# vr308/Generalised-Gaussian-Processes

Measured on AMD Instinct MI355X. Metric: ELBO evals/sec, higher is better.
Workload: dtype f64

## Files before the change

### generalised-gaussian-processes_amd/_lib.py

```python
from __future__ import annotations

import ctypes as C
import os

HERE = os.path.dirname(os.path.abspath(__file__))
LIB_PATH = os.path.join(HERE, "csrc", "libsgp_hip.so")

SGP_ABI_VERSION = 3
SGP_MAX_DIM = 32
SGP_MAX_INDUCING = 4096
KERNEL_IDS = {"rbf": 0, "matern32": 1, "matern52": 2, "composite": 3}
LIKELIHOOD_IDS = {"gaussian": 0, "bernoulli": 1, "bernoulli_logit": 2, "poisson": 3}
SGPMC_LIK_OUT_LEN = 3
COMP_LEN = 33
OPT_CONTRACTION, OPT_ASM_OVERLAP, OPT_KFU_BUDGET_BYTES, OPT_COND_LIMIT, OPT_CU_BUDGET, OPT_TIMING, OPT_SHARED_DEVICE = range(7)
OUT_F, OUT_LOGMARG, OUT_TRACE, OUT_LOGDETB, OUT_QUAD, OUT_TRW, OUT_S2BAR, OUT_KAPPABAR, OUT_LEN = range(9)


class SgpLibraryError(RuntimeError):
    pass


class SgpStatusError(RuntimeError):
    def __init__(self, fn, status, text):
        super().__init__("%s returned %d: %s" % (fn, status, text))
        self.status = status


_vp, _i64, _i32, _dbl, _sz = C.c_void_p, C.c_int64, C.c_int, C.c_double, C.c_size_t
_dp = C.POINTER(C.c_double)
_ip = C.POINTER(C.c_int)

PROTOTYPES = {
    "sgp_abi_version": (_i32, []),
    "sgp_status_string": (C.c_char_p, [_i32]),
    "sgp_ctx_create": (_vp, [_i32]),
    "sgp_ctx_destroy": (None, [_vp]),
    "sgp_ctx_device": (_i32, [_vp]),
    "sgp_ctx_set_option": (_i32, [_vp, _i32, _dbl]),
    "sgp_ctx_get_option": (_dbl, [_vp, _i32]),
    "sgp_ctx_bind_thread": (None, [_vp]),
    "sgp_ctx_set_pass1_gate": (None, [_vp, _vp]),
    "sgp_ctx_contraction_last": (_i32, [_vp]),
    "sgp_ctx_contraction_would_use_i8": (_i32, [_vp, _i64, _i32]),
    "sgp_ctx_timing_last_ms": (_i32, [_vp, _i32, C.POINTER(C.c_float)]),
    "sgp_ctx_timing_last_rows": (_i64, [_vp, _i32]),
    "sgp_ctx_suffstats_workspace_bytes": (_sz, [_vp, _i64, _i32, _i32, _i32]),
    "sgp_ctx_suffstats_fwd": (_i32, [_vp, _vp, _i64, _vp, _vp, _i64, _dp, _dbl, _i64, _i32, _i32, _i32,
                                     _vp, _vp, _vp, _vp, _vp, _vp, _sz, _vp]),
    "sgp_ctx_suffstats_bwd": (_i32, [_vp, _vp, _i64, _vp, _vp, _i64, _dp, _dbl, _vp, _vp, _dbl, _vp, _i64, _i32, _i32, _i32,
                                     _vp, _vp, _vp, _vp, _sz, _vp]),
    "sgp_ctx_kuu_factor": (_i32, [_vp, _vp, _i32, _vp, _vp, _vp, _sz, _vp]),
    "sgp_ctx_kuu_factor_ex": (_i32, [_vp, _vp, _i32, _vp, _vp, _vp, _vp, _sz, _vp]),
    "sgp_ctx_bound_from_stats": (_i32, [_vp, _vp, _vp, _vp, _vp, _vp, _dbl, _i64, _i32, _i32, _vp,
                                        _vp, _vp, _vp, _vp, _vp, _vp, _vp, _sz, _vp]),
    "sgp_ctx_suffstats_whitened_workspace_bytes": (_sz, [_vp, _i64, _i32, _i32]),
    "sgp_ctx_suffstats_fwd_whitened": (_i32, [_vp, _vp, _i64, _vp, _vp, _i64, _dp, _dbl, _i64, _i32, _i32, _i32, _vp,
                                              _vp, _vp, _vp, _vp, _vp, _sz, _vp]),
    "sgp_ctx_suffstats_whitened_rows_workspace_bytes": (_sz, [_vp, _i64, _i32, _i32, _i32]),
    "sgp_ctx_suffstats_fwd_whitened_rows": (_i32, [_vp, _vp, _i64, _vp, _vp, _i64, _dp, _dbl, _i64, _i32, _i32, _i32, _vp,
                                                   _vp, _vp, _vp, _vp, _vp, _vp, _sz, _vp]),
    "sgp_ctx_suffstats_extended_workspace_bytes": (_sz, [_vp, _i64, _i32, _i32]),
    "sgp_ctx_suffstats_fwd_extended": (_i32, [_vp, _vp, _i64, _vp, _vp, _i64, _dp, _dbl, _i64, _i32, _i32, _i32, _vp, _i32,
                                              _vp, _vp, _vp, _vp, _vp, _vp, _vp, _sz, _vp]),
    "sgp_ctx_suffstats_fwd_extended_f16": (_i32, [_vp, _vp, _i64, _vp, _vp, _i64, _dp, _dbl, _i64, _i32, _i32, _i32, _vp, _i32,
                                                  _vp, _vp, _vp, _vp, _vp, _vp, _vp, _vp, _sz, _vp]),
    "sgp_ctx_suffstats_bwd_factored_workspace_bytes": (_sz, [_vp, _i64, _i32, _i32, _i32]),
    "sgp_ctx_suffstats_bwd_factored": (_i32, [_vp, _vp, _i64, _vp, _vp, _i64, _dp, _dbl, _vp, _vp, _dbl, _vp, _dbl, _i64, _i32, _i32, _i32,
                                              _vp, _vp, _vp, _vp, _vp, _sz, _vp]),
    "sgp_ctx_bound_from_whitened_stats": (_i32, [_vp, _vp, _vp, _vp, _vp, _dbl, _i64, _i32, _i32, _vp,
                                                 _vp, _vp, _vp, _vp, _vp, _vp, _vp, _vp, _sz, _vp]),
    "sgp_ctx_mixture_predict": (_i32, [_vp, _vp, _i64, _vp, _i64, _vp, _i64, _i64, _vp, _i64, _i32, _dp, _dp, _dp, _dbl, _i32, _i32, _i32, _i32,
                                       _dbl, _vp, _vp, _vp, _vp, _vp, _vp, _sz, _vp]),
    "sgp_ctx_mixture_predict_zs": (_i32, [_vp, _vp, _i64, _vp, _i64, _vp, _i64, _i64, _vp, _i64, _i64, _i32, _dp, _dp, _dp, _dbl, _i32, _i32, _i32, _i32, _dbl, _vp, _vp, _vp, _vp, _vp, _vp, _sz, _vp]),
    "sgp_timing_enable": (None, [_i32]),
    "sgp_timing_last_ms": (_i32, [_i32, C.POINTER(C.c_float)]),
    "sgp_timing_last_rows": (_i64, [_i32]),
    "sgp_set_asm_overlap": (None, [_i32]),
    "sgp_set_cond_limit": (None, [_dbl]),
    "sgp_suffstats_workspace_bytes": (_sz, [_i64, _i32, _i32]),
    "sgp_suffstats_workspace_bytes_ex": (_sz, [_i64, _i32, _i32, _i32]),
    "sgp_suffstats_bwd_workspace_bytes_ex": (_sz, [_i64, _i32, _i32, _i32]),
    "sgp_kfu_len": (_sz, [_i64, _i32]),
    "sgp_set_kfu_budget_bytes": (None, [_sz]),
    "sgp_set_contraction": (_i32, [_i32]),
    "sgp_contraction_last": (_i32, []),
    "sgp_set_pass1_gate": (None, [_vp]),
    "sgp_suffstats_fwd": (_i32, [_vp, _i64, _vp, _vp, _i64, _dp, _dbl, _i64, _i32, _i32, _i32,
                                 _vp, _vp, _vp, _vp, _vp, _vp, _sz, _vp]),
    "sgp_stats_packed_len": (_sz, [_i32]),
    "sgp_stats_pack_lower": (_i32, [_vp, _i32, _vp, _vp]),
    "sgp_stats_unpack_lower": (_i32, [_vp, _i32, _vp, _vp]),
    "sgp_kuu": (_i32, [_vp, _i64, _dp, _dbl, _dbl, _i32, _i32, _i32, _vp, _vp]),
    "sgp_chol_workspace_bytes": (_sz, [_i32]),
    "sgp_chol_lower": (_i32, [_vp, _i64, _i32, _vp, _vp, _sz, _vp]),
    "sgp_trsm_workspace_bytes": (_sz, [_i32, _i32]),
    "sgp_trsm_lower": (_i32, [_vp, _i64, _vp, _i64, _i32, _i32, _i32, _vp, _sz, _vp]),
    "sgp_logdiag_sum": (_i32, [_vp, _i64, _i32, _vp, _vp]),
# ... 145 lines not shown
```

### generalised-gaussian-processes_amd/core.py

```python
from __future__ import annotations

import math

import torch

try:
    import torch.distributed as dist
except Exception:
    dist = None

from ._lib import COMP_LEN, OUT_F, OUT_LOGMARG, OUT_S2BAR, OUT_TRACE


class NotPositiveDefiniteError(RuntimeError):

    def __init__(self, info):
        super().__init__("matrix not positive definite: leading minor of order %d (1..M: Kuu, M+1..2M: B)" % info)
        self.info = info


class SgpTimeoutError(RuntimeError):

    def __init__(self):
        super().__init__("device time-out inside the dataflow Cholesky (SGP_INFO_TIMEOUT): outputs are invalid")
# ... 290 lines not shown
        if tier == TIER_WHITENED:
            self.guard.note_bound(ub, tol)
            return None
        need = required_tier(est, tol, reach, ext_ok)
        self.guard.note_exact(est, ub, tol)
        if need > tier:
            self.guard.open = True
            return need
        if info != 0:
            return tier + 1 if (tier + 1 < TIER_WHITENED and ext_ok) else TIER_WHITENED
        if strict and need < tier:
            return need
        return None

    def _forward(self, Z, ls, sf2, s2, with_adjoints, want_factors=False, extra=0, tier=TIER_STREAMING, report=False, want_lo=True):
        e = self.engine
        M = int(Z.shape[0])
        result = e.result_buffer(extra)
        if tier == TIER_EXTENDED:
            self.n_extended += 1
            Kuu = e.kuu(Z, ls, sf2, self.jitter, self.kernel)
            linv, _ = e.kuu_factor(Kuu, info=result[2], trace_out=self._trace_buf() if report else None)
            kfu = self._kfu_for(M) if with_adjoints else None
            diag = None
            if report:
                if self._phi_diag is None or self._phi_diag.numel() < M:
                    self._phi_diag = e.empty(M)
                diag = self._phi_diag
            dd = with_adjoints and self.extended_dd_phibar and hasattr(e, "phibar_dd")
            lo = dd and want_lo and kfu is not None and self._bwd_lo_ok(M)
            kfu_f16 = self._kfu_f16_for(M) if lo else None
            packed = e.suffstats_extended(self.X, self.y, Z, ls, sf2, linv, self.kernel, kfu=kfu, level=self.extended_level,
                                          **({"phi_diag": diag} if diag is not None else {}), **({"kfu_f16": kfu_f16} if kfu_f16 is not None else {}))
            self._allreduce_stats(packed, M)
            res = e.bound(Kuu, packed, s2, self.N, with_adjoints=with_adjoints, want_factors=want_factors, kuu_linv=linv,
                          result=result, whitened=True, **({"want_cw": True} if dd else {}))
            if dd:
                res["Phibar"], res["Phibar_lo"] = e.phibar_dd(res["Cw"], linv, s2, want_lo=lo)
                res["Cw"] = None
            if report:
                self._allreduce(diag[:M])
                e.streaming_error_report(diag, 1, self._trace_buf(), sf2, s2, self.N, M, result)
                res["reported"] = True
            res.update(packed=packed, kfu=kfu, kfu_f16=kfu_f16, t_keep=None, linv=linv)
            return res
        if tier == TIER_WHITENED:
            Kuu = e.kuu(Z, ls, sf2, self.jitter, self.kernel)
            rep = report and self.kernel != "composite"
            linv, _ = e.kuu_factor(Kuu, info=result[2], trace_out=self._trace_buf() if rep else None)
            factored = with_adjoints and self.factored_adjoint and hasattr(e, "suffstats_bwd_factored")
            t_keep = None
            if whitened_rows_layout(e, self.kernel, int(self.X.shape[0]), M, self.whitened_rows_min_work):
                t_keep = self._kfu_for(M) if factored else None
                packed = e.suffstats_whitened_rows(self.X, self.y, Z, ls, sf2, linv, self.kernel, t_out=t_keep)
            else:
                packed = e.suffstats_whitened(self.X, self.y, Z, ls, sf2, linv, self.kernel)
            self._allreduce_stats(packed, M)
            kw = {"want_cw": True} if factored else {}
            res = e.bound(Kuu, packed, s2, self.N, with_adjoints=with_adjoints, want_factors=want_factors, kuu_linv=linv,
                          result=result, whitened=True, **kw)
            if rep:
                e.streaming_error_report(None, 1, self._trace_buf(), sf2, s2, self.N, M, result)
                res["reported"] = True
            res.update(packed=packed, kfu=None, t_keep=t_keep, linv=linv)
            return res
        kfu = self._kfu_for(M) if with_adjoints else None
        gate = None
        guard = report
        trace = self._trace_buf() if guard and hasattr(e, "kuu_factor") else None
        overlap = (self.overlap_tail and hasattr(e, "kuu_factor") and e.device.type == "cuda"
                   and int(self.X.shape[0]) * M >= self.overlap_min_work)
        if overlap:
            main = torch.cuda.current_stream(e.device)
            side, (z_ready, ready), (Kuu, linv) = self._side_state(M)
            z_ready.record(main)
            side.wait_event(z_ready)
            e.kuu(Z, ls, sf2, self.jitter, self.kernel, out=Kuu, stream=side)
            e.kuu_factor(Kuu, info=result[2], trace_out=trace, out=linv, stream=side)
            ready.record(side)
            if (hasattr(e, "would_use_i8") and self.kernel != "composite" and int(self.X.shape[0]) >= 300 * M
                    and e.would_use_i8(int(self.X.shape[0]), M)):
                gate = ready
        try:
            packed = e.suffstats(self.X, self.y, Z, ls, sf2, self.kernel, kfu=kfu, **({"gate": gate} if gate is not None else {}))
            self._allreduce_stats(packed, M)
        finally:
            if overlap:
                main.wait_event(ready)
        if overlap:
            res = e.bound(Kuu, packed, s2, self.N, with_adjoints=with_adjoints, want_factors=want_factors, kuu_linv=linv,
                          result=result)
        elif guard and hasattr(e, "kuu_factor"):
            Kuu = e.kuu(Z, ls, sf2, self.jitter, self.kernel)
            linv, _ = e.kuu_factor(Kuu, info=result[2], trace_out=trace)
            res = e.bound(Kuu, packed, s2, self.N, with_adjoints=with_adjoints, want_factors=want_factors, kuu_linv=linv,
                          result=result)
        else:
            Kuu = e.kuu(Z, ls, sf2, self.jitter, self.kernel)
            res = e.bound(Kuu, packed, s2, self.N, with_adjoints=with_adjoints, want_factors=want_factors, result=result)
        if guard and trace is not None:
            e.streaming_error_report(packed, M + 1, trace, sf2, s2, self.N, M, result)
            res["reported"] = True
        res["packed"] = packed
        res["kfu"] = kfu
        return res

    def _pass2(self, res, Z, ls, sf2, s2, want_gz, g):
        e = self.engine
        if res.get("Cw") is not None:
            e.suffstats_bwd_factored(self.X, self.y, Z, ls, sf2, res["linv"], res["Cw"], s2, res["bbar"], -1.0 / (2.0 * float(s2)),
                                     self.kernel, want_gz=want_gz, out=g,
                                     **({"t_in": res["t_keep"]} if res.get("t_keep") is not None else {}))
        else:
            e.suffstats_bwd(self.X, self.y, Z, ls, sf2, res["Phibar"], res["bbar"], -1.0 / (2.0 * float(s2)),
                            self.kernel, want_gz=want_gz, out=g, kfu=res["kfu"])
            if res.get("Phibar_lo") is not None:
                n_lo = int(res.get("lo_slots", 0))
                e.suffstats_bwd_lo(self.X, self.y, Z, ls, sf2, res["Phibar_lo"], res["kfu"], g, self.kernel,
                                   **({"delta": g[g.numel() - n_lo:]} if n_lo else {}),
                                   **({"kfu_f16": res["kfu_f16"]} if res.get("kfu_f16") is not None else {}))
        if int(res.get("lo_slots", 0)) and res.get("Phibar_lo") is None:
            g[g.numel() - int(res["lo_slots"]):].zero_()
        self._allreduce(g)
        e.kuu_bwd(Z, ls, sf2, res["Kuubar"], g, self.kernel, want_gz=want_gz)

    def _evaluate(self, *args, **kw):
        try:
            return self._evaluate_once(*args, **kw)
        except SgpTimeoutError:
            e = self.engine
            if "shared_device" not in getattr(e, "OPTIONS", {}) or e.get_option("shared_device") != 0:
                raise
            e.set_option("shared_device", 1)
            self.n_timeout_retries += 1
            return self._evaluate_once(*args, **kw)

    def _evaluate_once(self, Z, ls, sf2, s2, with_grad=False, want_gz=False, want_factors=False, grad_reach=None, strict=False):
        e = self.engine
        M, d = int(Z.shape[0]), int(Z.shape[1])
        guard = self._guard_on(M)
        reach = self.extended_range
        if with_grad:
            reach = float(grad_reach) if grad_reach is not None else (self.extended_grad_range_lo if self._bwd_lo_ok(M) else self.extended_grad_range)
        ext_ok = self._extended_ok(M)
        if guard:
            tier = self.guard.start_tier(self.streaming_tol, reach, ext_ok)
            if strict and tier == TIER_WHITENED:
                tier = TIER_EXTENDED if ext_ok else TIER_STREAMING
            if tier != TIER_STREAMING:
                self.n_direct_whitened += 1
        else:
            tier = self._fixed_tier(M)
        nh = (e.hyper_len(self.kernel, d) if hasattr(e, "hyper_len") else d) if with_grad else 0
        lo_slots = (nh + 1) if (with_grad and guard and ext_ok and self._bwd_lo_ok(M)) else 0
        extra = nh + 1 + (M * d if want_gz else 0) + lo_slots if with_grad else 0
        if guard and with_grad and tier == TIER_EXTENDED and grad_reach is None and self._lo_skip > 0:
            self._lo_skip -= 1
            tier = TIER_WHITENED
        early = with_grad and self._rows_for_form * M >= self.early_check_min_work
        done = {}
        may_go_down = strict
        while True:
            res = self._forward(Z, ls, sf2, s2, with_adjoints=with_grad, want_factors=want_factors, extra=extra, tier=tier, report=guard,
                                want_lo=grad_reach is None)
            head = res["buf"].numel() - extra
            g = res["buf"][head:] if with_grad else None
            res["lo_slots"] = lo_slots
# ... 129 lines not shown
```

### generalised-gaussian-processes_amd/csrc/sgp_ctx.hip

```cpp
#include "sgp_common.hpp"
#include "sgp_ctx.hpp"
#include "sgp_stream.hpp"
#include <cstdlib>
#include <new>

namespace sgp {

static void ctx_init(Ctx& c, int device) {
  c.device = device;
  c.contraction = env_int("SGP_CONTRACTION", 1);
  if (c.contraction < 0 || c.contraction > 2) c.contraction = 1;
  c.asm_overlap = env_int("SGP_ASM_OVERLAP", 0);
  c.kfu_budget = KFU_BUDGET_DEFAULT;
  c.syrk_skip_upper = env_int("SGP_SYRK_SKIP_UPPER", 1);
  c.syrk_waves = env_int("SGP_SYRK_WAVES", 4);
  c.syrk_glds = env_int("SGP_SYRK_GLDS", 0);
  c.i8_prio = env_int("SGP_I8_PRIO", 0);
  c.shared_device = env_int("SGP_SHARED_DEVICE", 0) != 0 ? 1 : 0;
}

Ctx& default_ctx() {
  static Ctx* c = [] {
    Ctx* p = new Ctx();
    int dev = 0;
    if (hipGetDevice(&dev) != hipSuccess) dev = 0;
    ctx_init(*p, dev);
    return p;
  }();
  return *c;
}

static thread_local Ctx* t_cur = nullptr;
static thread_local Ctx* t_bound = nullptr;
Ctx& cur_ctx() { return t_cur ? *t_cur : (t_bound ? *t_bound : default_ctx()); }
void bind_thread_ctx(void* ctx) { t_bound = static_cast<Ctx*>(ctx); }
CtxScope::CtxScope(void* ctx) : prev(t_cur) { t_cur = ctx ? static_cast<Ctx*>(ctx) : &default_ctx(); }
CtxScope::~CtxScope() { t_cur = prev; }

}

using namespace sgp;

static bool ctx_on_current_device(const sgp_ctx* ctx) {
  if (!ctx) return true;
  int dev = -1;
  if (hipGetDevice(&dev) != hipSuccess) return true;
  return dev == reinterpret_cast<const Ctx*>(ctx)->device;
}

extern "C" sgp_ctx* sgp_ctx_create(int device) {
  if (device < 0) return nullptr;
  Ctx* c = new (std::nothrow) Ctx();
  if (!c) return nullptr;
  ctx_init(*c, device);
  return reinterpret_cast<sgp_ctx*>(c);
}

extern "C" void sgp_ctx_destroy(sgp_ctx* ctx) {
  if (!ctx) return;
  Ctx* c = reinterpret_cast<Ctx*>(ctx);
  if (c == &default_ctx()) return;
  if (c->ev_ready)
    for (int s = 0; s < CTX_TIMING_SLOTS; ++s)
      for (int k = 0; k < 2; ++k) (void)hipEventDestroy(c->ev[s][k]);
  if (c->side) {
    (void)hipStreamDestroy(c->side);
    (void)hipEventDestroy(c->ev_fork);
    (void)hipEventDestroy(c->ev_join);
  }
  delete c;
}

extern "C" int sgp_ctx_set_option(sgp_ctx* ctx, int option, double value) {
  Ctx& c = ctx ? *reinterpret_cast<Ctx*>(ctx) : default_ctx();
  switch (option) {
    case SGP_OPT_CONTRACTION:
      if (!(value >= 0.0 && value <= 2.0)) return SGP_ERR_ARG;
      c.contraction = (int)value;
      return SGP_OK;
    case SGP_OPT_ASM_OVERLAP:
      if (!(value >= 0.0 && value <= 2.0)) return SGP_ERR_ARG;
      c.asm_overlap = (int)value;
      return SGP_OK;
    case SGP_OPT_KFU_BUDGET_BYTES:
      if (!(value >= 0.0)) return SGP_ERR_ARG;
      c.kfu_budget = value > 0.0 ? (size_t)value : KFU_BUDGET_DEFAULT;
      return SGP_OK;
    case SGP_OPT_COND_LIMIT:
      c.cond_limit = value >= 0.0 ? value : 1e13;
      return SGP_OK;
    case SGP_OPT_CU_BUDGET:
      c.cu_budget = value > 0.0 ? (int)value : 0;
      return SGP_OK;
    case SGP_OPT_TIMING:
      c.timing = value != 0.0 ? 1 : 0;
      return SGP_OK;
    case SGP_OPT_SHARED_DEVICE:
      c.shared_device = value != 0.0 ? 1 : 0;
      return SGP_OK;
    default:
      return SGP_ERR_ARG;
  }
}

extern "C" double sgp_ctx_get_option(const sgp_ctx* ctx, int option) {
  const Ctx& c = ctx ? *reinterpret_cast<const Ctx*>(ctx) : default_ctx();
  switch (option) {
    case SGP_OPT_CONTRACTION: return (double)c.contraction;
    case SGP_OPT_ASM_OVERLAP: return (double)c.asm_overlap;
    case SGP_OPT_KFU_BUDGET_BYTES: return (double)c.kfu_budget;
    case SGP_OPT_COND_LIMIT: return c.cond_limit;
    case SGP_OPT_CU_BUDGET: return (double)c.cu_budget;
    case SGP_OPT_TIMING: return (double)c.timing;
    case SGP_OPT_SHARED_DEVICE: return (double)c.shared_device;
    default: return -1.0;
  }
}

extern "C" void sgp_ctx_bind_thread(sgp_ctx* ctx) { sgp::bind_thread_ctx(ctx); }

extern "C" int sgp_ctx_device(const sgp_ctx* ctx) { return (ctx ? *reinterpret_cast<const Ctx*>(ctx) : default_ctx()).device; }

extern "C" void sgp_ctx_set_pass1_gate(sgp_ctx* ctx, void* hip_event) {
  (ctx ? *reinterpret_cast<Ctx*>(ctx) : default_ctx()).pass1_gate = (hipEvent_t)hip_event;
}

extern "C" int sgp_ctx_contraction_last(const sgp_ctx* ctx) {
  return (ctx ? *reinterpret_cast<const Ctx*>(ctx) : default_ctx()).contraction_used;
}

extern "C" size_t sgp_ctx_suffstats_workspace_bytes(const sgp_ctx* ctx, int64_t N, int M, int d, int caller_owns_kfu) {
  CtxScope scope(const_cast<sgp_ctx*>(ctx));
  return sgp_suffstats_workspace_bytes_ex(N, M, d, caller_owns_kfu);
}
extern "C" int sgp_ctx_suffstats_fwd(sgp_ctx* ctx, const double* X, int64_t ldx, const double* y, const double* Z, int64_t ldz,
                                     const double* inv_ls, double sf2, int64_t N, int M, int d, int kernel_id, double* Phi, double* b,
                                     double* yy, double* kappa, double* Kfu_out, void* ws, size_t ws_bytes, sgp_stream_t stream) {
  if (!ctx_on_current_device(ctx)) return SGP_ERR_ARG;
  CtxScope scope(ctx);
  return sgp_suffstats_fwd(X, ldx, y, Z, ldz, inv_ls, sf2, N, M, d, kernel_id, Phi, b, yy, kappa, Kfu_out, ws, ws_bytes, stream);
}
extern "C" int sgp_ctx_suffstats_bwd(sgp_ctx* ctx, const double* X, int64_t ldx, const double* y, const double* Z, int64_t ldz,
                                     const double* inv_ls, double sf2, const double* Phibar, const double* bbar, double kappabar,
                                     const double* Kfu_in, int64_t N, int M, int d, int kernel_id, double* g_ls, double* g_sf2,
                                     double* g_Z, void* ws, size_t ws_bytes, sgp_stream_t stream) {
  if (!ctx_on_current_device(ctx)) return SGP_ERR_ARG;
  CtxScope scope(ctx);
  return sgp_suffstats_bwd(X, ldx, y, Z, ldz, inv_ls, sf2, Phibar, bbar, kappabar, Kfu_in, N, M, d, kernel_id, g_ls, g_sf2, g_Z, ws,
                           ws_bytes, stream);
}
extern "C" int sgp_ctx_kuu_factor(sgp_ctx* ctx, const double* Kuu, int M, double* Linv_out, int* info, void* ws, size_t ws_bytes,
                                  sgp_stream_t stream) {
  if (!ctx_on_current_device(ctx)) return SGP_ERR_ARG;
  CtxScope scope(ctx);
  return sgp_kuu_factor(Kuu, M, Linv_out, info, ws, ws_bytes, stream);
}
extern "C" int sgp_ctx_kuu_factor_ex(sgp_ctx* ctx, const double* Kuu, int M, double* Linv_out, int* info, double* trace_out, void* ws,
                                     size_t ws_bytes, sgp_stream_t stream) {
  if (!ctx_on_current_device(ctx)) return SGP_ERR_ARG;
  CtxScope scope(ctx);
  return sgp_kuu_factor_ex(Kuu, M, Linv_out, info, trace_out, ws, ws_bytes, stream);
}
extern "C" int sgp_ctx_bound_from_stats(sgp_ctx* ctx, const double* Kuu, const double* Phi, const double* b, const double* yy,
                                        const double* kappa, double s2, int64_t N, int M, int with_adjoints, double* out,
                                        double* Phibar, double* bbar, double* Kuubar, double* factors, const double* kuu_linv,
                                        int* info, void* ws, size_t ws_bytes, sgp_stream_t stream) {
  if (!ctx_on_current_device(ctx)) return SGP_ERR_ARG;
  CtxScope scope(ctx);
  return sgp_bound_from_stats(Kuu, Phi, b, yy, kappa, s2, N, M, with_adjoints, out, Phibar, bbar, Kuubar, factors, kuu_linv, info, ws,
                              ws_bytes, stream);
}
extern "C" int sgp_ctx_mixture_predict(sgp_ctx* ctx, const double* X, int64_t ldx, const double* y, int64_t N, const double* Xs,
                                       int64_t ldxs, int64_t T, const double* Z, int64_t ldz, int S, const double* inv_ls,
                                       const double* sf2, const double* s2, double jitter, int M, int d, int kernel_id, int pred_noise,
                                       double gate_jitter, double* mean, double* var, double* cov, int* info, int* gate_info, void* ws,
                                       size_t ws_bytes, sgp_stream_t stream) {
  if (!ctx_on_current_device(ctx)) return SGP_ERR_ARG;
  CtxScope scope(ctx);
  return sgp_mixture_predict(X, ldx, y, N, Xs, ldxs, T, Z, ldz, S, inv_ls, sf2, s2, jitter, M, d, kernel_id, pred_noise, gate_jitter,
                             mean, var, cov, info, gate_info, ws, ws_bytes, stream);
}

extern "C" size_t sgp_ctx_suffstats_whitened_workspace_bytes(const sgp_ctx* ctx, int64_t N, int M, int d) {
  CtxScope scope(const_cast<sgp_ctx*>(ctx));
  return sgp_suffstats_whitened_workspace_bytes(N, M, d);
}
extern "C" int sgp_ctx_suffstats_fwd_whitened(sgp_ctx* ctx, const double* X, int64_t ldx, const double* y, const double* Z, int64_t ldz,
                                              const double* inv_ls, double sf2, int64_t N, int M, int d, int kernel_id,
                                              const double* kuu_linv, double* W, double* u, double* yy, double* kappa, void* ws,
                                              size_t ws_bytes, sgp_stream_t stream) {
  if (!ctx_on_current_device(ctx)) return SGP_ERR_ARG;
  CtxScope scope(ctx);
  return sgp_suffstats_fwd_whitened(X, ldx, y, Z, ldz, inv_ls, sf2, N, M, d, kernel_id, kuu_linv, W, u, yy, kappa, ws, ws_bytes, stream);
}
extern "C" size_t sgp_ctx_suffstats_whitened_rows_workspace_bytes(const sgp_ctx* ctx, int64_t N, int M, int d, int caller_owns_t) {
  CtxScope scope(const_cast<sgp_ctx*>(ctx));
  return sgp_suffstats_whitened_rows_workspace_bytes(N, M, d, caller_owns_t);
// ... 82 lines not shown
```

### generalised-gaussian-processes_amd/csrc/sgp_ctx.hpp

```cpp
#pragma once
#include <hip/hip_runtime.h>
#include <cstddef>
#include <cstdint>

namespace sgp {

constexpr int CTX_TIMING_SLOTS = 3;

struct Ctx {
  int device = 0;
  int contraction = 1;
  int asm_overlap = 0;
  size_t kfu_budget = 0;
  double cond_limit = 1e13;
  int cu_budget = 0;
  int timing = 0;
  int shared_device = 0;
  int syrk_skip_upper = 1, syrk_waves = 4, syrk_glds = 0, i8_prio = 0;
  int contraction_used = 0;
  hipEvent_t pass1_gate = nullptr;
  int64_t syrk_timed_rows = 0;
  hipEvent_t ev[CTX_TIMING_SLOTS][2] = {};
  int ev_ready = 0, ev_used[CTX_TIMING_SLOTS] = {0, 0, 0};
  hipStream_t side = nullptr;
  hipEvent_t ev_fork = nullptr, ev_join = nullptr;
};

Ctx& default_ctx();
Ctx& cur_ctx();

void bind_thread_ctx(void* ctx);

struct CtxScope {
  Ctx* prev;
  explicit CtxScope(void* ctx);
  ~CtxScope();
  CtxScope(const CtxScope&) = delete;
  CtxScope& operator=(const CtxScope&) = delete;
};

}
```

### generalised-gaussian-processes_amd/csrc/sgp_stream.hpp

```cpp
#pragma once
#include <cstdlib>
#include <initializer_list>
#include <type_traits>
#include "sgp_common.hpp"

namespace sgp {

constexpr int TILE = 128;
constexpr int NB = 16;
constexpr int KROW = 2 * TILE + 16;
constexpr int ASM_ROWS = 256;
constexpr int TARGET_WGS = 2048;
constexpr int RESIDENT_WGS = 512;
constexpr size_t KFU_BUDGET_DEFAULT = size_t(16) << 30;
size_t stream_kfu_budget();

static inline int dp_for(int d) {
  const int opts[] = {2, 4, 8, 16, 24, 32};
  for (int o : opts)
    if (d <= o) return o;
  return -1;
}

struct StreamPlan {
  int Mp, ntr, ntiles, DP;
  int64_t Npad;
  int asm_sub;
  int64_t sc_rows;
  int nsplit;
  int taper[4];
  int nmb;
  int nsplit_b;
  int taper_b[4];
};

static inline int64_t bpart_rows(const StreamPlan& p) { return p.Npad / ASM_ROWS > 0 ? p.Npad / ASM_ROWS * p.asm_sub : 1; }

struct SplitMap {
  int g[4];
  int cps;
};
__host__ __device__ inline void split_range(const SplitMap& m, int split, int64_t nchunks, int64_t& c0, int64_t& c1) {
  const int64_t groups = (int64_t)m.g[0] + m.g[1] + m.g[2] + m.g[3];
  if (groups == 0) {
    c0 = (int64_t)split * m.cps;
    c1 = c0 + m.cps;
    if (c1 > nchunks) c1 = nchunks;
    if (c0 > nchunks) c0 = nchunks;
    return;
  }
  const int64_t total = 8 * (8 * (int64_t)m.g[0] + 4 * (int64_t)m.g[1] + 2 * (int64_t)m.g[2] + (int64_t)m.g[3]);
  int64_t gg = split >> 3, before = 0;
  int w = 8;
  for (int l = 0; l < 4; ++l) {
    if (gg >= m.g[l]) {
      before += (int64_t)m.g[l] * 8 * w;
      gg -= m.g[l];
      w >>= 1;
    } else {
      before += gg * 8 * w;
      break;
    }
  }
  if (w == 0) w = 1;
  const int64_t cum0 = before + (int64_t)(split & 7) * w;
  c0 = cum0 * nchunks / total;
  c1 = (cum0 + w) * nchunks / total;
}

static inline SplitMap split_map(const int* taper, int64_t nchunks, int nsplit) {
  const int cps = (int)((nchunks + nsplit - 1) / nsplit);
  SplitMap m{{0, 0, 0, 0}, cps < 1 ? 1 : cps};
  for (int l = 0; taper && l < 4; ++l) m.g[l] = taper[l];
  return m;
}

static inline StreamPlan make_stream_plan(int64_t N, int M, int d) {
  StreamPlan p;
  p.Mp = padded_m(M);
  p.ntr = p.Mp / TILE;
  p.ntiles = p.ntr * (p.ntr + 1) / 2;
  p.DP = dp_for(d);
  p.Npad = N > 0 ? round_up64(N, ASM_ROWS) : 0;
  {
    const int64_t base = (p.Npad / ASM_ROWS) * ((p.Mp + 255) / 256);
    p.asm_sub = base < 128 ? 8 : (base < 256 ? 4 : 1);
  }
  static const int asm_sub_override = env_int("SGP_ASM_SUB", 0);
  if (asm_sub_override == 1 || asm_sub_override == 4 || asm_sub_override == 8 || asm_sub_override == 16) p.asm_sub = asm_sub_override;
  int64_t cap = (int64_t)(stream_kfu_budget() / ((size_t)p.Mp * 8)) / ASM_ROWS * ASM_ROWS;
  if (cap < ASM_ROWS) cap = ASM_ROWS;
  p.sc_rows = p.Npad < cap ? p.Npad : cap;
  const int64_t nchunks = p.sc_rows / NB;
  static const int target_wgs = env_int("SGP_TARGET_WGS", TARGET_WGS);
  const bool target_wgs_set = getenv("SGP_TARGET_WGS") != nullptr;
  int64_t k = (target_wgs + 8 * p.ntiles - 1) / (8 * p.ntiles);
  int64_t ns = 8 * k;
  if (nchunks >= 64 * 8 && !target_wgs_set) {
    double best_waste = 2.0;
    for (int64_t kk = (3072 + 8 * p.ntiles - 1) / (8 * p.ntiles); 8 * kk * p.ntiles <= 5632; ++kk) {
      const int64_t cand = 8 * kk;
      if (kk < 1 || nchunks / cand < 64) break;
      const double r = (double)p.ntiles * (double)cand / (double)RESIDENT_WGS;
      const double rounds = (double)(int64_t)(r + 0.999999);
      const double waste = (rounds - r) / rounds;
      if (waste < best_waste - 1e-9) {
        best_waste = waste;
        ns = cand;
      }
    }
  }
  if (nchunks / ns < 16 && !target_wgs_set) {
    int64_t one_round = 8 * ((RESIDENT_WGS * 4 / 5) / (8 * p.ntiles));
    if (one_round < 8) one_round = 8;
    if (one_round < ns) ns = one_round;
  }
  static const int ns_override = env_int("SGP_SYRK_NSPLIT", 0);
  if (ns_override > 0) ns = 8 * ((ns_override + 7) / 8);
  const int64_t lim = round_up64(nchunks > 0 ? nchunks : 1, 8);
  if (ns > lim) ns = lim;
  p.nsplit = (int)ns;
  p.taper[0] = p.taper[1] = p.taper[2] = p.taper[3] = 0;
  static const int taper_on = env_int("SGP_SYRK_TAPER", 1);
  if (taper_on && !target_wgs_set && ns % 32 == 0 && nchunks / ns >= 64) {
    const int B = (int)(ns / 8);
    p.taper[0] = 3 * B / 4; p.taper[1] = B / 4; p.taper[2] = B / 4; p.taper[3] = B / 2;
    p.nsplit = 8 * (p.taper[0] + p.taper[1] + p.taper[2] + p.taper[3]);
  }
  p.nmb = p.Mp / TILE;
  const int64_t nblocks = p.sc_rows / TILE;
  int64_t nsb = 8 * ((TARGET_WGS + 8 * p.nmb - 1) / (8 * p.nmb));
  if (nblocks / nsb < 2) {
    const int64_t one_round = 8 * ((RESIDENT_WGS + 8 * p.nmb - 1) / (8 * p.nmb));
    if (one_round < nsb) nsb = one_round;
  }
  static const int nsb_override = env_int("SGP_KBAR_NSPLIT", 0);
  if (nsb_override > 0) nsb = 8 * ((nsb_override + 7) / 8);
  const int64_t limb = round_up64(nblocks > 0 ? nblocks : 1, 8);
  if (nsb > limb) nsb = limb;
  p.nsplit_b = (int)nsb;
  p.taper_b[0] = p.taper_b[1] = p.taper_b[2] = p.taper_b[3] = 0;
  static const int taper_b_on = env_int("SGP_KBAR_TAPER", 1);
  if (taper_b_on && nsb % 32 == 0 && nblocks / nsb >= 8) {
    const int B = (int)(nsb / 8);
    p.taper_b[0] = 3 * B / 4; p.taper_b[1] = B / 4; p.taper_b[2] = B / 4; p.taper_b[3] = B / 2;
    p.nsplit_b = 8 * (p.taper_b[0] + p.taper_b[1] + p.taper_b[2] + p.taper_b[3]);
  }
  return p;
}

static inline int check_stream_args(std::initializer_list<const void*> required, const double* X, int64_t ldx, const double* y, int64_t ldz,
                                    int64_t N, int M, int d, int kernel_id, bool composite_ok) {
  for (const void* ptr : required)
    if (!ptr) return SGP_ERR_ARG;
  if (N < 0 || M <= 0 || d <= 0 || ldz < d) return SGP_ERR_ARG;
  if (N > 0 && (!X || !y || ldx < d)) return SGP_ERR_ARG;
  if (kernel_id < 0 || kernel_id > SGP_KERNEL_COMPOSITE || (kernel_id == SGP_KERNEL_COMPOSITE && !composite_ok)) return SGP_ERR_ARG;
  if (d > SGP_MAX_DIM || M > SGP_MAX_INDUCING) return SGP_ERR_DIM;
  return SGP_OK;
}
static inline bool stream_shape_ok(int64_t N, int M, int d) { return N >= 0 && M > 0 && d > 0 && d <= SGP_MAX_DIM && M <= SGP_MAX_INDUCING; }

struct SuperChunks {
  int64_t Npad, step;
  struct Range { int64_t r0, rows; };
  struct It {
    int64_t r0, Npad, step;
    Range operator*() const { return {r0, Npad - r0 < step ? Npad - r0 : step}; }
    void operator++() { r0 += step; }
    bool operator!=(const It&) const { return r0 < Npad; }
  };
  It begin() const { return {0, Npad, step}; }
  It end() const { return {Npad, Npad, step}; }
};

template <typename F>
static inline void dispatch_dp(int DP, F&& f) {
  switch (DP) {
    case 2: f(std::integral_constant<int, 2>()); break;
    case 4: f(std::integral_constant<int, 4>()); break;
    case 8: f(std::integral_constant<int, 8>()); break;
    case 16: f(std::integral_constant<int, 16>()); break;
    case 24: f(std::integral_constant<int, 24>()); break;
    default: f(std::integral_constant<int, 32>()); break;
  }
}

enum { TIMING_ASSEMBLE = 0, TIMING_SYRK = 1, TIMING_KBAR = 2, TIMING_SLOTS = 3 };
void timing_begin(int slot, hipStream_t st);
void timing_end(int slot, hipStream_t st);

struct PadSymJob {
  const double* P = nullptr;
  double* out = nullptr;
  const double* vec = nullptr;
  double* vout = nullptr;
};
void stream_prologue(const StreamPlan& p, const KernArgs& ka, const double* X, int64_t ldx, const double* y,
                     const double* Z, int64_t ldz, int64_t N, int M, double* Xs, double* ys, double* Zs, double* yypart,
                     hipStream_t st, const PadSymJob& pad = PadSymJob());
void stream_assemble(const StreamPlan& p, int kid, const double* Xs, const double* ys, const double* Zs, int64_t row0,
                     int64_t rows, int64_t N, int M, double* Kfu, double* bpart, hipStream_t st);

struct Ctx;
struct FwdWs {
  double *Xs, *ys, *Zs, *Kfu, *slab, *bpart, *btmp, *yypart;
  uint8_t* Q;
  size_t bytes;
};
FwdWs carve_fwd(void* ws, const StreamPlan& p, bool need_kfu, int64_t qrows);
struct WhRowsWs {
  FwdWs f;
  double *R, *T;
  size_t bytes;
};
WhRowsWs carve_wh_rows(void* ws, const StreamPlan& p, bool caller_t);
void launch_syrk(const Ctx& cx, const double* K, int Mp, int64_t nchunks, const SplitMap& smap, int ntiles, int nsplit, int accum,
                 double* slab, hipStream_t st);
void reduce_slabs(const StreamPlan& p, const double* slab, int nslabs, int M, double scale, double* out, hipStream_t st);
void launch_tpart(const double* T, const double* ys, int64_t row0, int64_t rows, int Mp, double* bpart, hipStream_t st);
void reduce_bparts(const StreamPlan& p, const double* bpart, double* btmp, const double* yypart, int nparts, double sf2, int64_t N, int M,
                   double* b, double* yy, double* kappa, hipStream_t st);

constexpr int I8_SPLIT_ROWS = 16384;
static inline int i8_nsplit(int64_t rows, int Mp) {
  const int nrt = Mp / 128, ntiles = nrt * (nrt + 1);
  int64_t lo = (rows + I8_SPLIT_ROWS - 1) / I8_SPLIT_ROWS;
  lo = (lo + 7) / 8 * 8;
  if (lo < 8) lo = 8;
  int64_t best = lo;
  double best_waste = 2.0;
  for (int64_t cand = lo; cand <= 2 * lo + 8; cand += 8) {
    if (cand > lo && rows / cand < 2048) break;
    const double r = (double)ntiles * (double)cand / 256.0;
    const double rounds = (double)(int64_t)(r + 0.999999);
    const double waste = (rounds - r) / rounds;
    if (waste < best_waste - 1e-9) {
      best_waste = waste;
      best = cand;
    }
  }
  return (int)best;
}
__host__ __device__ inline void i8_split_steps(int64_t nsteps, int nsplit, int split, int64_t& c0, int64_t& c1) {
  const int64_t per = (nsteps + nsplit - 1) / nsplit;
  c0 = (int64_t)split * per;
  c1 = c0 + per;
  if (c0 > nsteps) c0 = nsteps;
  if (c1 > nsteps) c1 = nsteps;
}
void i8_assemble(const StreamPlan& p, int kid, const double* Xs, const double* ys, const double* Zs, int64_t row0, int64_t rows,
                 int64_t N, int M, uint8_t* Q, double* Kfu , double* bpart, hipStream_t st,
                 uint16_t* Kh = nullptr );
int i8_contract(const uint8_t* Q, int Mp, int64_t rows, int nsplit, int accumulate, double* slab, hipStream_t st, double* slab_lo = nullptr,
                int level = 1);

}
```

### generalised-gaussian-processes_amd/csrc/sgp_suffstats_bwd.hip

```cpp
#include "sgp_common.hpp"
#include "sgp_stream.hpp"
#include "sgp_composite.hpp"
#include "sgp_dense.hpp"
#include <cstdlib>

namespace sgp {

constexpr int BK = 16;
constexpr int ALD = BK + 2;
constexpr int BROW = TILE + 16;
constexpr int A_DBL = TILE * ALD;
constexpr int B_DBL = BK * BROW;
constexpr int BSM = 2 * (A_DBL + B_DBL);
constexpr int CS = 129;
static_assert(64 * CS <= BSM, "epilogue image must fit in the main-loop buffers");

__global__ void bwd_pad_vec_kernel(const double* __restrict__ in, int64_t n, int64_t npad, double* __restrict__ out) {
  for (int64_t i = (int64_t)blockIdx.x * blockDim.x + threadIdx.x; i < npad; i += (int64_t)gridDim.x * blockDim.x)
    out[i] = i < n ? in[i] : 0.0;
}
__global__ void bwd_pad_plain_kernel(const double* __restrict__ P, int M, int Mp, double scale, double* __restrict__ out) {
  const int64_t total = (int64_t)Mp * Mp;
  for (int64_t e = (int64_t)blockIdx.x * blockDim.x + threadIdx.x; e < total; e += (int64_t)gridDim.x * blockDim.x) {
    const int r = (int)(e / Mp), c = (int)(e - (int64_t)r * Mp);
    out[e] = (r < M && c < M) ? scale * P[e] : 0.0;
  }
}
__global__ void bwd_pad_small_kernel(const double* __restrict__ P, int M, int Mp, double scale, double* __restrict__ out) {
  const int64_t total = (int64_t)Mp * Mp;
  for (int64_t e = (int64_t)blockIdx.x * blockDim.x + threadIdx.x; e < total; e += (int64_t)gridDim.x * blockDim.x) {
    const int r = (int)(e / Mp), c = (int)(e - (int64_t)r * Mp);
    out[e] = (r < M && c < M) ? scale * P[(int64_t)r * M + c] : 0.0;
  }
}

template <int KID>
__device__ __forceinline__ double hprime_from_k(double kp, double r2) {
  if constexpr (KID == SGP_KERNEL_RBF) {
    return -0.5 * kp;
  } else if constexpr (KID == SGP_KERNEL_MATERN32) {
    const double a = 1.7320508075688772 * sqrt(r2);
    return -1.5 * kp / (1.0 + a);
  } else {
    const double a = 2.23606797749979 * sqrt(r2);
    return -(5.0 / 6.0) * (1.0 + a) * kp / (1.0 + a + a * a * (1.0 / 3.0));
  }
}

template <int DP, int KID, bool KP>
constexpr bool kbar_two_pass() {
#ifdef SGP_AB_KBAR_TWO_PASS_ALL
  return KP && KID == SGP_KERNEL_RBF;
#else
  return KP && DP > 8 && KID == SGP_KERNEL_RBF;
#endif
}

#ifdef SGP_AB_KBAR_UNROLL4
#define SGP_KBAR_EPI_UNROLL _Pragma("unroll 4")
#else
#define SGP_KBAR_EPI_UNROLL _Pragma("unroll 2")
#endif

template <int DP, int KID, bool GZ, bool KP = true>
__global__ __launch_bounds__(256, ((DP <= 8 || kbar_two_pass<DP, KID, KP>()) ? 2 : 1)) void kbar_contract_kernel(
    const double* __restrict__ Kfu, const double* __restrict__ Xs, const double* __restrict__ ys,
    const double* __restrict__ Zs, const double* __restrict__ Pb, const double* __restrict__ bb, double sf2,
    int64_t row0, int64_t nblocks, SplitMap bmap, int64_t N, int M, int Mp, int nmb, int want_gz, int accumulate,
    double* __restrict__ gacc, double* __restrict__ gzpart, double* __restrict__ glpart) {
  __shared__ double smem[BSM];
  double (*At)[TILE][ALD] = reinterpret_cast<double (*)[TILE][ALD]>(smem);
  double (*Bt)[BK][BROW] = reinterpret_cast<double (*)[BK][BROW]>(smem + 2 * A_DBL);
  double (*Ct)[CS] = reinterpret_cast<double (*)[CS]>(smem);

  const int xcd = blockIdx.x & 7;
  const int jj = blockIdx.x >> 3;
  const int mb = jj % nmb;
  const int split = (jj / nmb) * 8 + xcd;
  int64_t nb0, nb1;
  split_range(bmap, split, nblocks, nb0, nb1);
  const int m0 = mb * TILE;

  const int tid = threadIdx.x, lane = tid & 63;
  const int wave = __builtin_amdgcn_readfirstlane(tid >> 6);
  const int wi = wave >> 1, wj = wave & 1, l15 = lane & 15, l4 = lane >> 4;
  const int half = wave >> 1;
// ... 194 lines not shown
    }
#pragma unroll
    for (int j = 0; j < DP; ++j) {
      gmine[(size_t)j * 256] = gl[j];
      if (want_gz) gmine[(size_t)(DP + j) * 256] = gz[j];
    }
    gmine[(size_t)(2 * DP) * 256] = gs;
    }
  }

  double gl[DP], gz[DP], gs;
  {
    const bool any = nb0 < nb1;
#pragma unroll
    for (int j = 0; j < DP; ++j) {
      gl[j] = any ? gmine[(size_t)j * 256] : 0.0;
      gz[j] = (any && want_gz) ? gmine[(size_t)(DP + j) * 256] : 0.0;
    }
    gs = any ? gmine[(size_t)(2 * DP) * 256] : 0.0;
  }
  double* scratch = smem;
  if (want_gz) {
#pragma unroll
    for (int j = 0; j < DP; ++j) {
      __syncthreads();
      if (half == 1) scratch[erow] = gz[j];
      __syncthreads();
      if (half == 0) {
        double* dst = gzpart + ((size_t)split * Mp + m0 + erow) * DP + j;
        const double v = gz[j] + scratch[erow];
        *dst = accumulate ? *dst + v : v;
      }
    }
  }
  auto block_total = [&](double v, int slot) {
    v = wave_sum(v);
    __syncthreads();
    if (lane == 0) scratch[wave] = v;
    __syncthreads();
    if (tid == 0) {
      double* dst = glpart + ((size_t)split * nmb + mb) * (DP + 1) + slot;
      const double t = scratch[0] + scratch[1] + scratch[2] + scratch[3];
      *dst = accumulate ? *dst + t : t;
    }
  };
#pragma unroll
  for (int j = 0; j < DP; ++j) block_total(gl[j], j);
  block_total(gs, DP);
}

__global__ __launch_bounds__(256) void bwd_reduce_kernel(const double* __restrict__ gzpart, const double* __restrict__ glpart,
                                                         int nsplit, int nmb, int Mp, int M, int DP, KernArgs ka,
                                                         double kappa_term, double* __restrict__ g_ls,
                                                         double* __restrict__ g_sf2, double* __restrict__ g_Z) {
  const int d = ka.d;
  if (blockIdx.x == 0) {
    const int np = nsplit * nmb;
    const int lane = threadIdx.x & 63, wave = threadIdx.x >> 6;
    for (int q = wave; q <= d; q += 4) {
      const int j = q == d ? DP : q;
      double s = 0.0;
      for (int p = lane; p < np; p += 64) s += glpart[(size_t)p * (DP + 1) + j];
      s = wave_sum(s);
      if (lane == 0) {
        if (q == d) *g_sf2 = s + kappa_term;
        else g_ls[q] = -2.0 * ka.inv_ls[q] * s;
      }
    }
  }
  if (g_Z) {
    const int64_t total = (int64_t)M * d;
    for (int64_t e = (int64_t)blockIdx.x * 256 + threadIdx.x; e < total; e += (int64_t)gridDim.x * 256) {
      const int m = (int)(e / d), j = (int)(e - (int64_t)m * d);
      double s = 0.0;
#pragma unroll 8
      for (int sp = 0; sp < nsplit; ++sp) s += gzpart[((size_t)sp * Mp + m) * DP + j];
      g_Z[e] = 2.0 * ka.inv_ls[j] * s;
    }
  }
}

struct BwdWs {
  double *Xs, *ys, *Zs, *Pb, *bb, *gzpart, *glpart, *gacc, *bpart, *yypart, *Kfu;
  size_t bytes;
};
static BwdWs carve_bwd(void* ws, const StreamPlan& p, bool need_kfu) {
  Carver c(ws);
  BwdWs w;
  w.Xs = c.take<double>((size_t)(p.Npad > 0 ? p.Npad : 1) * p.DP);
  w.ys = c.take<double>((size_t)(p.Npad > 0 ? p.Npad : 1));
  w.Zs = c.take<double>((size_t)p.Mp * p.DP);
  w.Pb = c.take<double>((size_t)p.Mp * p.Mp);
  w.bb = c.take<double>((size_t)p.Mp);
  w.gzpart = c.take<double>((size_t)p.nsplit_b * p.Mp * p.DP);
  w.glpart = c.take<double>((size_t)p.nsplit_b * p.nmb * (p.DP + 1));
  w.gacc = c.take<double>((size_t)p.nsplit_b * p.nmb * (2 * p.DP + 1) * 256);
  w.bpart = c.take<double>((size_t)bpart_rows(p) * p.Mp);
  w.yypart = c.take<double>(256);
  w.Kfu = need_kfu ? c.take<double>((size_t)(p.sc_rows > 0 ? p.sc_rows : 1) * p.Mp) : nullptr;
  w.bytes = c.used();
  return w;
}

template <bool KP>
static void launch_kbar(const StreamPlan& p, int kid, const double* K, const BwdWs& w, double sf2, int64_t row0, int64_t nblocks, int64_t N,
                        int M, int want_gz, int accumulate, hipStream_t st) {
  const int grid = p.nmb * p.nsplit_b;
  const SplitMap bmap = split_map(p.taper_b, nblocks, p.nsplit_b);
#define SGP_BWD_ARGS K, w.Xs, w.ys, w.Zs, w.Pb, w.bb, sf2, row0, nblocks, bmap, N, M, p.Mp, p.nmb, want_gz, accumulate, w.gacc, w.gzpart, w.glpart
#define SGP_BWD_LAUNCH(KID) \
  do { \
    if (want_gz) kbar_contract_kernel<DP, KID, true, KP><<<grid, 256, 0, st>>>(SGP_BWD_ARGS); \
    else kbar_contract_kernel<DP, KID, false, KP><<<grid, 256, 0, st>>>(SGP_BWD_ARGS); \
  } while (0)
  dispatch_dp(p.DP, [&](auto dp) {
    constexpr int DP = decltype(dp)::value;
    switch (kid) {
      case SGP_KERNEL_RBF: SGP_BWD_LAUNCH(SGP_KERNEL_RBF); break;
      case SGP_KERNEL_MATERN32: SGP_BWD_LAUNCH(SGP_KERNEL_MATERN32); break;
      default: SGP_BWD_LAUNCH(SGP_KERNEL_MATERN52); break;
    }
  });
#undef SGP_BWD_LAUNCH
#undef SGP_BWD_ARGS
}
static void finish_grads(const StreamPlan& p, const BwdWs& w, const KernArgs& ka, double kappabar, int64_t N, int M, double* g_ls,
                         double* g_sf2, double* g_Z, hipStream_t st) {
  const int64_t tot = (int64_t)M * ka.d;
  const int rg = (int)((tot + 255) / 256 < 1024 ? (tot + 255) / 256 : 1024);
  bwd_reduce_kernel<<<rg < 1 ? 1 : rg, 256, 0, st>>>(w.gzpart, w.glpart, p.nsplit_b, p.nmb, p.Mp, M, p.DP, ka, kappabar * (double)N, g_ls,
                                                    g_sf2, g_Z);
}

}

using namespace sgp;

static size_t bwd_workspace_bytes(int64_t N, int M, int d, bool library_kfu) {
  if (!stream_shape_ok(N, M, d)) return 0;
  StreamPlan p = make_stream_plan(N, M, d);
  const size_t fast = carve_bwd(nullptr, p, library_kfu).bytes;
  const size_t comp = d <= COMP_MAX_DIM ? comp_bwd_workspace_bytes(N, M, d) : 0;
  return fast > comp ? fast : comp;
}
extern "C" size_t sgp_suffstats_bwd_workspace_bytes(int64_t N, int M, int d) { return bwd_workspace_bytes(N, M, d, true); }
extern "C" size_t sgp_suffstats_bwd_workspace_bytes_ex(int64_t N, int M, int d, int caller_owns_kfu) {
  return bwd_workspace_bytes(N, M, d, caller_owns_kfu == 0);
}

extern "C" int sgp_suffstats_bwd(const double* X, int64_t ldx, const double* y, const double* Z, int64_t ldz,
                                 const double* inv_ls, double sf2, const double* Phibar, const double* bbar,
                                 double kappabar, const double* Kfu_in, int64_t N, int M, int d, int kernel_id,
                                 double* g_ls, double* g_sf2, double* g_Z, void* ws, size_t ws_bytes,
                                 sgp_stream_t stream) {
  if (const int bad = check_stream_args({Z, inv_ls, Phibar, bbar, g_ls, g_sf2}, X, ldx, y, ldz, N, M, d, kernel_id, true)) return bad;
  if (kernel_id == SGP_KERNEL_COMPOSITE) {
    CompSpec cs;
    if (comp_parse(inv_ls, d, &cs) != SGP_OK) return SGP_ERR_ARG;
    fill_zero(g_sf2, 1, (hipStream_t)stream);
    return comp_suffstats_bwd(X, ldx, y, Z, ldz, cs, Phibar, bbar, kappabar, N, M, d, g_ls, g_Z, ws, ws_bytes, (hipStream_t)stream);
  }
  StreamPlan p = make_stream_plan(N, M, d);
  if (Kfu_in) p.sc_rows = p.Npad;
  BwdWs w = carve_bwd(ws, p, Kfu_in == nullptr);
  if (!ws || ws_bytes < w.bytes) return SGP_ERR_WORKSPACE;
  hipStream_t st = (hipStream_t)stream;
  const KernArgs ka = make_kern_args(inv_ls, sf2, d);
  {
    PadSymJob pad;
    pad.P = Phibar; pad.out = w.Pb; pad.vec = bbar; pad.vout = w.bb;
    stream_prologue(p, ka, X, ldx, y, Z, ldz, N, M, w.Xs, w.ys, w.Zs, w.yypart, st, pad);
  }

  const int want_gz = g_Z != nullptr;
  if (p.Npad == 0) launch_kbar<true>(p, kernel_id, nullptr, w, sf2, 0, 0, N, M, want_gz, 0, st);
  for (auto [r0, rows] : SuperChunks{p.Npad, p.sc_rows}) {
    const double* Kfu = Kfu_in ? Kfu_in + r0 * p.Mp : nullptr;
    if (!Kfu_in) {
      stream_assemble(p, kernel_id, w.Xs, w.ys, w.Zs, r0, rows, N, M, w.Kfu, w.bpart, st);
      Kfu = w.Kfu;
    }
    timing_begin(TIMING_KBAR, st);
    launch_kbar<true>(p, kernel_id, Kfu, w, sf2, r0, rows / TILE, N, M, want_gz, r0 > 0 ? 1 : 0, st);
    timing_end(TIMING_KBAR, st);
  }
  finish_grads(p, w, ka, kappabar, N, M, g_ls, g_sf2, g_Z, st);
  return check_launch();
}

static int bwd_fully_factored() {
  static const int v = env_int("SGP_BWD_FULLY_FACTORED", 0);
  return v;
}
static size_t bwd_factored_workspace_bytes(int64_t N, int M, int d, bool caller_t) {
  if (!stream_shape_ok(N, M, d)) return 0;
  StreamPlan p = make_stream_plan(N, M, d);
  p.sc_rows = p.Npad;
  const int nt = (caller_t ? 0 : 1) + (bwd_fully_factored() ? 1 : 0);
  const size_t fast = carve_bwd(nullptr, p, !caller_t).bytes + nt * round_up64((int64_t)(p.Npad > 0 ? p.Npad : 1) * p.Mp * 8 + 256, 256) +
                      3 * round_up64((int64_t)p.Mp * p.Mp * 8 + 256, 256);
  const size_t comp = d <= COMP_MAX_DIM ? comp_bwd_factored_workspace_bytes(N, M, d) : 0;
  return fast > comp ? fast : comp;
}
extern "C" size_t sgp_suffstats_bwd_factored_workspace_bytes(int64_t N, int M, int d) { return bwd_factored_workspace_bytes(N, M, d, false); }
extern "C" size_t sgp_suffstats_bwd_factored_workspace_bytes_ex(int64_t N, int M, int d, int caller_owns_t) {
  return bwd_factored_workspace_bytes(N, M, d, caller_owns_t != 0);
}

static int bwd_factored(const double* X, int64_t ldx, const double* y, const double* Z, int64_t ldz, const double* inv_ls, double sf2,
                        const double* kuu_linv, const double* Cw, double s2, const double* bbar, double kappabar, int64_t N, int M,
                        int d, int kernel_id, const double* T_in, double* g_ls, double* g_sf2, double* g_Z, void* ws, size_t ws_bytes,
                        sgp_stream_t stream) {
  if (!(s2 > 0.0) || (T_in && kernel_id == SGP_KERNEL_COMPOSITE)) return SGP_ERR_ARG;
  if (const int bad = check_stream_args({Z, inv_ls, kuu_linv, Cw, bbar, g_ls, g_sf2}, X, ldx, y, ldz, N, M, d, kernel_id, true)) return bad;
  hipStream_t st = (hipStream_t)stream;
  if (!ws || ws_bytes < bwd_factored_workspace_bytes(N, M, d, T_in != nullptr)) return SGP_ERR_WORKSPACE;
  if (kernel_id == SGP_KERNEL_COMPOSITE) {
    CompSpec cs;
    if (comp_parse(inv_ls, d, &cs) != SGP_OK) return SGP_ERR_ARG;
    fill_zero(g_sf2, 1, st);
    return comp_suffstats_bwd_factored(X, ldx, y, Z, ldz, cs, kuu_linv, Cw, s2, bbar, kappabar, N, M, d, g_ls, g_Z, ws, ws_bytes, st);
  }
  const int fully = bwd_fully_factored();
  StreamPlan p = make_stream_plan(N, M, d);
  p.sc_rows = p.Npad;
  BwdWs w = carve_bwd(ws, p, T_in == nullptr);
  Carver c(static_cast<char*>(ws) + round_up64((int64_t)w.bytes, 256));
  const size_t rows = (size_t)(p.Npad > 0 ? p.Npad : 1);
  double* T1 = T_in ? nullptr : c.take<double>(rows * p.Mp);
  double* T2 = fully ? c.take<double>(rows * p.Mp) : nullptr;
  double* P2 = c.take<double>((size_t)p.Mp * p.Mp);
  double* Q0 = c.take<double>((size_t)p.Mp * p.Mp);
  double* R = c.take<double>((size_t)p.Mp * p.Mp);
  const KernArgs ka = make_kern_args(inv_ls, sf2, d);
  stream_prologue(p, ka, X, ldx, y, Z, ldz, N, M, w.Xs, w.ys, w.Zs, w.yypart, st);
  bwd_pad_plain_kernel<<<2048, 256, 0, st>>>(kuu_linv, M, p.Mp, 0.5, fully ? w.Pb : Q0);
  bwd_pad_small_kernel<<<2048, 256, 0, st>>>(Cw, M, p.Mp, 1.0 / s2, P2);
  if (!fully) {
    GemmDesc q;
    q.A = P2; q.lda = p.Mp; q.B = Q0; q.ldb = p.Mp; q.C = w.Pb; q.ldc = p.Mp;
    q.m = p.Mp; q.n = p.Mp; q.k = p.Mp; q.klo_mask = 2;
    gemm(q, st);
  }
  bwd_pad_vec_kernel<<<(p.Mp + 255) / 256, 256, 0, st>>>(bbar, M, p.Mp, w.bb);
  const int want_gz = g_Z != nullptr;
  const double* T1c = T_in ? T_in : T1;
  if (p.Npad > 0) {
    if (!T_in) {
      stream_assemble(p, kernel_id, w.Xs, w.ys, w.Zs, 0, p.Npad, N, M, w.Kfu, w.bpart, st);
      transpose_square(kuu_linv, p.Mp, R, st);
      GemmDesc g1;
      g1.A = w.Kfu; g1.lda = p.Mp; g1.B = R; g1.ldb = p.Mp; g1.C = T1; g1.ldc = p.Mp;
      g1.m = (int)p.Npad; g1.n = p.Mp; g1.k = p.Mp;
      g1.khi_mask = 2;
      gemm(g1, st);
    }
    if (fully) {
// ... 28 lines not shown
```

### generalised-gaussian-processes_amd/csrc/sgp_suffstats_fwd.hip

```cpp
#include "sgp_common.hpp"
#include "sgp_stream.hpp"
#include "sgp_dense.hpp"
#include "sgp_composite.hpp"
#include "sgp_ctx.hpp"
#include <cstdlib>

namespace sgp {

static_assert(TIMING_SLOTS == CTX_TIMING_SLOTS, "timing slots");
size_t stream_kfu_budget() { return cur_ctx().kfu_budget; }

void timing_begin(int slot, hipStream_t st) {
  Ctx& c = cur_ctx();
  if (!c.timing) return;
  if (!c.ev_ready) {
    bool ok = true;
    for (int s = 0; s < TIMING_SLOTS; ++s)
      for (int k = 0; k < 2; ++k) ok = (hipEventCreate(&c.ev[s][k]) == hipSuccess) && ok;
    if (!ok) return;
    c.ev_ready = 1;
  }
  if (hipEventRecord(c.ev[slot][0], st) != hipSuccess) c.ev_used[slot] = 0;
}
void timing_end(int slot, hipStream_t st) {
// ... 388 lines not shown
    }
  }
}

template <int DP, int ROWS>
static void launch_assemble_rows(int kid, dim3 grid, hipStream_t st, const double* Xs, const double* ys, const double* Zs,
                                 int64_t row0, int64_t N, int M, int Mp, double* Kfu, double* bpart) {
  switch (kid) {
    case SGP_KERNEL_RBF: kfu_assemble_kernel<DP, SGP_KERNEL_RBF, ROWS><<<grid, 256, 0, st>>>(Xs, ys, Zs, row0, N, M, Mp, Kfu, bpart); break;
    case SGP_KERNEL_MATERN32: kfu_assemble_kernel<DP, SGP_KERNEL_MATERN32, ROWS><<<grid, 256, 0, st>>>(Xs, ys, Zs, row0, N, M, Mp, Kfu, bpart); break;
    default: kfu_assemble_kernel<DP, SGP_KERNEL_MATERN52, ROWS><<<grid, 256, 0, st>>>(Xs, ys, Zs, row0, N, M, Mp, Kfu, bpart); break;
  }
}
template <int DP>
static void launch_assemble(int kid, int sub, dim3 grid, hipStream_t st, const double* Xs, const double* ys, const double* Zs,
                            int64_t row0, int64_t N, int M, int Mp, double* Kfu, double* bpart) {
  if (sub == 16) launch_assemble_rows<DP, ASM_ROWS / 16>(kid, grid, st, Xs, ys, Zs, row0, N, M, Mp, Kfu, bpart);
  else if (sub == 8) launch_assemble_rows<DP, ASM_ROWS / 8>(kid, grid, st, Xs, ys, Zs, row0, N, M, Mp, Kfu, bpart);
  else if (sub == 4) launch_assemble_rows<DP, ASM_ROWS / 4>(kid, grid, st, Xs, ys, Zs, row0, N, M, Mp, Kfu, bpart);
  else launch_assemble_rows<DP, ASM_ROWS>(kid, grid, st, Xs, ys, Zs, row0, N, M, Mp, Kfu, bpart);
}

void stream_assemble(const StreamPlan& p, int kid, const double* Xs, const double* ys, const double* Zs, int64_t row0,
                     int64_t rows, int64_t N, int M, double* Kfu, double* bpart, hipStream_t st) {
  dim3 grid((unsigned)(rows / ASM_ROWS * p.asm_sub), (p.Mp + 255) / 256);
  dispatch_dp(p.DP, [&](auto dp) { launch_assemble<decltype(dp)::value>(kid, p.asm_sub, grid, st, Xs, ys, Zs, row0, N, M, p.Mp, Kfu, bpart); });
}

void stream_prologue(const StreamPlan& p, const KernArgs& ka, const double* X, int64_t ldx, const double* y,
                     const double* Z, int64_t ldz, int64_t N, int M, double* Xs, double* ys, double* Zs, double* yypart,
                     hipStream_t st, const PadSymJob& pad) {
  int gx = 0;
  if (N > 0) {
    const int64_t tot = p.Npad * p.DP;
    gx = (int)((tot + 255) / 256 < 4096 ? (tot + 255) / 256 : 4096);
  }
  const int gz = (p.Mp * p.DP + 255) / 256;
  int gp = 0;
  if (pad.P) {
    const int64_t blocks = ((int64_t)p.Mp * p.Mp + 255) / 256;
    gp = (int)(blocks < 2048 ? blocks : 2048);
  }
  stream_prologue_kernel<<<gx + gz + 256 + gp, 256, 0, st>>>(X, ldx, N, p.Npad, Z, ldz, M, p.Mp, p.DP, ka, Xs, Zs, y, ys, yypart, gx, gz, pad, gp);
}

static int syrk_grid(int nsplit, int ntiles) { return 8 * ((nsplit >> 3) * ntiles + (((nsplit & 7) * ntiles + 7) >> 3)); }

constexpr int HEAD_SPLITS_MAX = 24;
static bool side_stream_ready(Ctx& c) {
  if (c.side) return true;
  int lo = 0, hi = 0;
  if (hipDeviceGetStreamPriorityRange(&lo, &hi) != hipSuccess) return false;
  if (hipStreamCreateWithPriority(&c.side, hipStreamNonBlocking, hi) != hipSuccess) { c.side = nullptr; return false; }
  if (hipEventCreateWithFlags(&c.ev_fork, hipEventDisableTiming) != hipSuccess ||
      hipEventCreateWithFlags(&c.ev_join, hipEventDisableTiming) != hipSuccess) {
    (void)hipStreamDestroy(c.side);
    c.side = nullptr;
    return false;
  }
  return true;
}
static void head_block(const StreamPlan& p, int64_t nchunks, int* head_ns, int64_t* head_chunks) {
  *head_ns = 0;
  *head_chunks = 0;
  const int g_asm_overlap = cur_ctx().asm_overlap;
  int hs = RESIDENT_WGS / p.ntiles;
  if (hs > HEAD_SPLITS_MAX) hs = HEAD_SPLITS_MAX;
  const int64_t w = 8 * (int64_t)p.taper[0] + 4 * p.taper[1] + 2 * p.taper[2] + p.taper[3];
  if (g_asm_overlap == 0 || hs < 8 || w == 0 || p.sc_rows != p.Npad) return;
  int64_t c = nchunks / (w + hs);
  int64_t nh = (hs * c) / (ASM_ROWS / NB) * (ASM_ROWS / NB);
  if (c < 64 || nh <= 0 || nh * 4 > nchunks) return;
  *head_ns = hs;
  *head_chunks = nh;
}

constexpr double I8_MIN_WORK = 4294967296.0;

static int contraction_mode() { return cur_ctx().contraction; }
static bool i8_rule(int mode, int64_t Npad, int Mp) {
  return Npad > 0 && (mode == 2 || (mode == 1 && (double)Npad * Mp * Mp >= I8_MIN_WORK));
}

constexpr int BRED_G = 64;
FwdWs carve_fwd(void* ws, const StreamPlan& p, bool need_kfu, int64_t qrows) {
  Carver c(ws);
  FwdWs w;
  w.Xs = c.take<double>((size_t)(p.Npad > 0 ? p.Npad : 1) * p.DP);
  w.ys = c.take<double>((size_t)(p.Npad > 0 ? p.Npad : 1));
  w.Zs = c.take<double>((size_t)p.Mp * p.DP);
  int nslab = p.nsplit + HEAD_SPLITS_MAX;
  if (qrows > 0 && i8_nsplit(qrows, p.Mp) > nslab) nslab = i8_nsplit(qrows, p.Mp);
  w.slab = c.take<double>((size_t)nslab * p.ntiles * TILE * TILE);
  w.bpart = c.take<double>((size_t)bpart_rows(p) * p.Mp);
  w.btmp = c.take<double>((size_t)BRED_G * p.Mp);
  w.yypart = c.take<double>(256);
  w.Kfu = need_kfu ? c.take<double>((size_t)(p.sc_rows > 0 ? p.sc_rows : 1) * p.Mp) : nullptr;
  const bool own_q = !need_kfu && i8_rule(contraction_mode(), p.Npad, p.Mp);
  w.Q = need_kfu ? reinterpret_cast<uint8_t*>(w.Kfu) : (own_q ? c.take<uint8_t>((size_t)(qrows > 0 ? qrows : 1) * p.Mp * 7) : nullptr);
  w.bytes = c.used();
  return w;
}

void launch_syrk(const Ctx& cx, const double* K, int Mp, int64_t nchunks, const SplitMap& smap, int ntiles, int nsplit, int accum,
                        double* slab, hipStream_t st) {
  const int skip_upper = cx.syrk_skip_upper;
  const int nwaves = cx.syrk_waves, glds = cx.syrk_glds;
  const int g = syrk_grid(nsplit, ntiles);
#define SGP_SYRK_LAUNCH(NWV, GL, SK) \
  syrk_tile_kernel<NWV, GL, SK><<<g, NWV * 64, 0, st>>>(K, Mp, nchunks, smap, ntiles, accum, slab, nsplit)
  if (glds) {
    if (skip_upper) SGP_SYRK_LAUNCH(4, true, true); else SGP_SYRK_LAUNCH(4, true, false);
  } else if (nwaves == 8) {
    if (skip_upper) SGP_SYRK_LAUNCH(8, false, true); else SGP_SYRK_LAUNCH(8, false, false);
  } else {
    if (skip_upper) SGP_SYRK_LAUNCH(4, false, true); else SGP_SYRK_LAUNCH(4, false, false);
  }
#undef SGP_SYRK_LAUNCH
}
static void zero_slabs(const StreamPlan& p, const double* K, double* slab, hipStream_t st) {
  syrk_tile_kernel<4, false, false><<<p.ntiles * p.nsplit, 256, 0, st>>>(K, p.Mp, 0, split_map(nullptr, 0, p.nsplit), p.ntiles, 0, slab, p.nsplit);
}

void reduce_bparts(const StreamPlan& p, const double* bpart, double* btmp, const double* yypart, int nparts, double sf2, int64_t N, int M,
                   double* b, double* yy, double* kappa, hipStream_t st) {
  bpart_stage1_kernel<<<dim3(p.Mp / 64, BRED_G), 256, 0, st>>>(bpart, p.Npad / ASM_ROWS * nparts, p.Mp, BRED_G, btmp);
  finalize_stats_kernel<<<(M + 255) / 256, 256, 0, st>>>(btmp, BRED_G, p.Mp, M, yypart, 256, sf2, sf2 * (double)N, b, yy, kappa);
}
template <typename Ws>
static void finish_b(const StreamPlan& p, const Ws& w, int nparts, double sf2, int64_t N, int M, double* b, double* yy, double* kappa,
                     hipStream_t st) {
  reduce_bparts(p, w.bpart, w.btmp, w.yypart, nparts, sf2, N, M, b, yy, kappa, st);
}
void reduce_slabs(const StreamPlan& p, const double* slab, int nslabs, int M, double scale, double* Phi, hipStream_t st) {
  const int nb32 = p.Mp / 32;
  reduce_phi_kernel<<<nb32 * (nb32 + 1) / 2, 256, 0, st>>>(slab, nslabs, p.ntiles, M, scale, Phi);
}
static void finish_stats(const StreamPlan& p, const FwdWs& w, int nslabs, int nparts, double sf2, int64_t N, int M, double* Phi, double* b,
                         double* yy, double* kappa, hipStream_t st) {
  reduce_slabs(p, w.slab, nslabs, M, sf2 * sf2, Phi, st);
  finish_b(p, w, nparts, sf2, N, M, b, yy, kappa, st);
}

__global__ __launch_bounds__(256) void tpart_kernel(const double* __restrict__ T, const double* __restrict__ ys, int64_t row0, int Mp,
                                                    double* __restrict__ bpart) {
  __shared__ double ysh[ASM_ROWS];
  const int64_t rbase = (int64_t)blockIdx.x * ASM_ROWS;
  ysh[threadIdx.x] = ys[row0 + rbase + threadIdx.x];
  __syncthreads();
  const int m = blockIdx.y * 256 + threadIdx.x;
  if (m >= Mp) return;
  const double* src = T + (size_t)rbase * Mp + m;
  double a0 = 0.0, a1 = 0.0, a2 = 0.0, a3 = 0.0;
#pragma unroll 2
  for (int i = 0; i < ASM_ROWS; i += 4) {
    a0 = fma(__builtin_nontemporal_load(src + (size_t)i * Mp), ysh[i], a0);
    a1 = fma(__builtin_nontemporal_load(src + (size_t)(i + 1) * Mp), ysh[i + 1], a1);
    a2 = fma(__builtin_nontemporal_load(src + (size_t)(i + 2) * Mp), ysh[i + 2], a2);
    a3 = fma(__builtin_nontemporal_load(src + (size_t)(i + 3) * Mp), ysh[i + 3], a3);
  }
  bpart[((row0 + rbase) / ASM_ROWS) * Mp + m] = (a0 + a1) + (a2 + a3);
}
void launch_tpart(const double* T, const double* ys, int64_t row0, int64_t rows, int Mp, double* bpart, hipStream_t st) {
  tpart_kernel<<<dim3((unsigned)(rows / ASM_ROWS), (Mp + 255) / 256), 256, 0, st>>>(T, ys, row0, Mp, bpart);
}

// ... 186 lines not shown
  w.Zs = c.take<double>((size_t)p.Mp * p.DP);
  w.slab = c.take<double>(ns);
  w.slab_lo = c.take<double>(ns);
  w.bpart = c.take<double>((size_t)bpart_rows(p) * p.Mp);
  w.btmp = c.take<double>((size_t)BRED_G * p.Mp);
  w.yypart = c.take<double>(256);
  w.Ph = c.take<double>(mm); w.Pl = c.take<double>(mm);
  w.Yh = c.take<double>(mm); w.Yl = c.take<double>(mm);
  w.Wh = c.take<double>(mm); w.Wl = c.take<double>(mm);
  w.bpad = c.take<double>(p.Mp);
  w.upad = c.take<double>(p.Mp);
  w.Q = c.take<uint8_t>((size_t)(qrows > 0 ? qrows : 1) * p.Mp * 7);
  w.bytes = c.used();
  return w;
}

WhRowsWs carve_wh_rows(void* ws, const StreamPlan& p, bool caller_t) {
  WhRowsWs w;
  w.f = carve_fwd(ws, p, true, 0);
  Carver c(ws ? static_cast<char*>(ws) + round_up64((int64_t)w.f.bytes, 256) : nullptr);
  w.R = c.take<double>((size_t)p.Mp * p.Mp);
  w.T = caller_t ? nullptr : c.take<double>((size_t)(p.sc_rows > 0 ? p.sc_rows : 1) * p.Mp);
  w.bytes = (size_t)round_up64((int64_t)w.f.bytes, 256) + c.used();
  return w;
}

}

using namespace sgp;

static int ctx_timing_last_ms(Ctx& c, int slot, float* ms) {
  if (slot < 0 || slot >= TIMING_SLOTS || !ms) return SGP_ERR_ARG;
  if (!c.ev_ready || !c.ev_used[slot]) return SGP_ERR_ARG;
  if (hipEventSynchronize(c.ev[slot][1]) != hipSuccess) return SGP_ERR_LAUNCH;
  return hipEventElapsedTime(ms, c.ev[slot][0], c.ev[slot][1]) == hipSuccess ? SGP_OK : SGP_ERR_LAUNCH;
}
extern "C" int sgp_ctx_timing_last_ms(sgp_ctx* ctx, int slot, float* ms) {
  return ctx_timing_last_ms(ctx ? *reinterpret_cast<Ctx*>(ctx) : default_ctx(), slot, ms);
}
extern "C" int64_t sgp_ctx_timing_last_rows(const sgp_ctx* ctx, int slot) {
  return slot == TIMING_SYRK ? (ctx ? *reinterpret_cast<const Ctx*>(ctx) : default_ctx()).syrk_timed_rows : -1;
}
extern "C" int sgp_ctx_contraction_would_use_i8(const sgp_ctx* ctx, int64_t N, int M) {
  if (N <= 0 || M <= 0 || M > SGP_MAX_INDUCING) return 0;
  return i8_rule((ctx ? *reinterpret_cast<const Ctx*>(ctx) : default_ctx()).contraction, round_up64(N, ASM_ROWS), padded_m(M)) ? 1 : 0;
}

extern "C" void sgp_timing_enable(int on) { default_ctx().timing = on ? 1 : 0; }
extern "C" int sgp_timing_last_ms(int slot, float* ms) { return ctx_timing_last_ms(default_ctx(), slot, ms); }
extern "C" int64_t sgp_timing_last_rows(int slot) { return sgp_ctx_timing_last_rows(nullptr, slot); }
extern "C" void sgp_set_asm_overlap(int mode) { default_ctx().asm_overlap = (mode < 0 || mode > 2) ? 0 : mode; }
extern "C" int sgp_set_contraction(int mode) {
  const int prev = default_ctx().contraction;
  default_ctx().contraction = (mode < 0 || mode > 2) ? 1 : mode;
  return prev;
}
extern "C" int sgp_contraction_last(void) { return default_ctx().contraction_used; }
extern "C" void sgp_set_pass1_gate(void* hip_event) { default_ctx().pass1_gate = (hipEvent_t)hip_event; }
extern "C" void sgp_set_kfu_budget_bytes(size_t bytes) { default_ctx().kfu_budget = bytes ? bytes : KFU_BUDGET_DEFAULT; }

extern "C" size_t sgp_kfu_len(int64_t N, int M) {
  if (N < 0 || M <= 0 || M > SGP_MAX_INDUCING) return 0;
  return (size_t)round_up64(N > 0 ? N : 1, ASM_ROWS) * padded_m(M);
}

static size_t fwd_workspace_bytes(int64_t N, int M, int d, bool library_kfu) {
  if (!stream_shape_ok(N, M, d)) return 0;
  StreamPlan p = make_stream_plan(N, M, d);
  const size_t fast = carve_fwd(nullptr, p, library_kfu, p.sc_rows).bytes, comp = comp_fwd_workspace_bytes(N, M);
  return fast > comp ? fast : comp;
}
extern "C" size_t sgp_suffstats_workspace_bytes(int64_t N, int M, int d) { return fwd_workspace_bytes(N, M, d, true); }
extern "C" size_t sgp_suffstats_workspace_bytes_ex(int64_t N, int M, int d, int caller_owns_kfu) {
  return fwd_workspace_bytes(N, M, d, caller_owns_kfu == 0);
}

extern "C" int sgp_suffstats_fwd(const double* X, int64_t ldx, const double* y, const double* Z, int64_t ldz,
                                 const double* inv_ls, double sf2, int64_t N, int M, int d, int kernel_id,
                                 double* Phi, double* b, double* yy, double* kappa, double* Kfu_out, void* ws,
                                 size_t ws_bytes, sgp_stream_t stream) {
  Ctx& cx = cur_ctx();
  hipEvent_t gate = cx.pass1_gate;
  cx.pass1_gate = nullptr;
  if (const int bad = check_stream_args({Z, inv_ls, Phi, b, yy, kappa}, X, ldx, y, ldz, N, M, d, kernel_id, true)) return bad;
  if (kernel_id == SGP_KERNEL_COMPOSITE) {
    CompSpec cs;
    if (comp_parse(inv_ls, d, &cs) != SGP_OK) return SGP_ERR_ARG;
    return comp_suffstats_fwd(X, ldx, y, Z, ldz, cs, N, M, d, Phi, b, yy, kappa, ws, ws_bytes, (hipStream_t)stream);
  }
  StreamPlan p = make_stream_plan(N, M, d);
  const int64_t qrows = p.sc_rows;
  if (Kfu_out) p.sc_rows = p.Npad;
  FwdWs w = carve_fwd(ws, p, Kfu_out == nullptr, qrows);
  if (!ws || ws_bytes < w.bytes) return SGP_ERR_WORKSPACE;
  hipStream_t st = (hipStream_t)stream;
  stream_prologue(p, make_kern_args(inv_ls, sf2, d), X, ldx, y, Z, ldz, N, M, w.Xs, w.ys, w.Zs, w.yypart, st);
  double* Kfu = Kfu_out ? Kfu_out : w.Kfu;
  if (p.Npad == 0) zero_slabs(p, Kfu, w.slab, st);
  auto contract = [&](const double* K, int64_t nchunks, const SplitMap& smap, int nsplit, int accum, double* slab) {
    launch_syrk(cx, K, p.Mp, nchunks, smap, p.ntiles, nsplit, accum, slab, st);
  };
  int nslabs = p.nsplit;
  int head_ns = 0;
  int64_t head_chunks = 0;
  const bool use_i8 = i8_rule(cx.contraction, p.Npad, p.Mp);
  cx.contraction_used = use_i8 ? 1 : 0;
  if (!use_i8) gate = nullptr;
  if (p.Npad > 0 && !use_i8) head_block(p, p.Npad / NB, &head_ns, &head_chunks);
  if (use_i8) {
    const int ns = i8_nsplit(qrows, p.Mp);
    for (auto [r0, rows] : SuperChunks{p.Npad, qrows}) {
      timing_begin(TIMING_ASSEMBLE, st);
      i8_assemble(p, kernel_id, w.Xs, w.ys, w.Zs, r0, rows, N, M, w.Q, Kfu_out ? Kfu_out + (size_t)r0 * p.Mp : nullptr, w.bpart, st);
      timing_end(TIMING_ASSEMBLE, st);
      if (gate && hipStreamWaitEvent(st, gate, 0) != hipSuccess) return SGP_ERR_LAUNCH;
      gate = nullptr;
      timing_begin(TIMING_SYRK, st);
      if (i8_contract(w.Q, p.Mp, rows, ns, r0 > 0 ? 1 : 0, w.slab, st) != SGP_OK) return SGP_ERR_LAUNCH;
      timing_end(TIMING_SYRK, st);
      cx.syrk_timed_rows = rows;
    }
    nslabs = ns;
  } else if (head_ns > 0) {
    const int64_t hrows = head_chunks * NB, trows = p.Npad - hrows, tchunks = trows / NB;
    const bool side = cx.asm_overlap == 1 && side_stream_ready(cx);
    double* head_slab = w.slab + (size_t)p.nsplit * p.ntiles * TILE * TILE;
    const SplitMap hmap = split_map(nullptr, head_chunks, head_ns), tmap = split_map(p.taper, tchunks, p.nsplit);
    timing_begin(TIMING_ASSEMBLE, st);
    stream_assemble(p, kernel_id, w.Xs, w.ys, w.Zs, 0, hrows, N, M, Kfu, w.bpart, st);
    bool forked = false;
    if (side && hipEventRecord(cx.ev_fork, st) == hipSuccess && hipStreamWaitEvent(cx.side, cx.ev_fork, 0) == hipSuccess) {
      stream_assemble(p, kernel_id, w.Xs, w.ys, w.Zs, hrows, trows, N, M, Kfu + (size_t)hrows * p.Mp, w.bpart, cx.side);
      forked = hipEventRecord(cx.ev_join, cx.side) == hipSuccess;
      if (!forked) (void)hipStreamSynchronize(cx.side);
    } else {
      stream_assemble(p, kernel_id, w.Xs, w.ys, w.Zs, hrows, trows, N, M, Kfu + (size_t)hrows * p.Mp, w.bpart, st);
    }
    timing_end(TIMING_ASSEMBLE, st);
    contract(Kfu, head_chunks, hmap, head_ns, 0, head_slab);
    if (forked && hipStreamWaitEvent(st, cx.ev_join, 0) != hipSuccess) (void)hipStreamSynchronize(cx.side);
    timing_begin(TIMING_SYRK, st);
    contract(Kfu + (size_t)hrows * p.Mp, tchunks, tmap, p.nsplit, 0, w.slab);
    timing_end(TIMING_SYRK, st);
    cx.syrk_timed_rows = trows;
    nslabs = p.nsplit + head_ns;
  } else {
    for (auto [r0, rows] : SuperChunks{p.Npad, p.sc_rows}) {
      timing_begin(TIMING_ASSEMBLE, st);
      stream_assemble(p, kernel_id, w.Xs, w.ys, w.Zs, r0, rows, N, M, Kfu, w.bpart, st);
      timing_end(TIMING_ASSEMBLE, st);
      timing_begin(TIMING_SYRK, st);
      contract(Kfu, rows / NB, split_map(p.taper, rows / NB, p.nsplit), p.nsplit, r0 > 0 ? 1 : 0, w.slab);
      timing_end(TIMING_SYRK, st);
      cx.syrk_timed_rows = rows;
    }
  }
  finish_stats(p, w, nslabs, use_i8 ? 1 : p.asm_sub, sf2, N, M, Phi, b, yy, kappa, st);
  return check_launch();
}

extern "C" size_t sgp_suffstats_whitened_rows_workspace_bytes(int64_t N, int M, int d, int caller_owns_t) {
  if (!stream_shape_ok(N, M, d)) return 0;
  StreamPlan p = make_stream_plan(N, M, d);
  if (caller_owns_t) p.sc_rows = p.Npad;
  return carve_wh_rows(nullptr, p, caller_owns_t != 0).bytes;
}
extern "C" int sgp_suffstats_fwd_whitened_rows(const double* X, int64_t ldx, const double* y, const double* Z, int64_t ldz,
                                               const double* inv_ls, double sf2, int64_t N, int M, int d, int kernel_id,
                                               const double* kuu_linv, double* W, double* u, double* yy, double* kappa, double* T_out,
                                               void* ws, size_t ws_bytes, sgp_stream_t stream) {
  Ctx& cx = cur_ctx();
  if (const int bad = check_stream_args({Z, inv_ls, kuu_linv, W, u, yy, kappa}, X, ldx, y, ldz, N, M, d, kernel_id, false)) return bad;
  StreamPlan p = make_stream_plan(N, M, d);
  if (T_out) p.sc_rows = p.Npad;
  WhRowsWs w = carve_wh_rows(ws, p, T_out != nullptr);
  if (!ws || ws_bytes < w.bytes) return SGP_ERR_WORKSPACE;
  hipStream_t st = (hipStream_t)stream;
  stream_prologue(p, make_kern_args(inv_ls, sf2, d), X, ldx, y, Z, ldz, N, M, w.f.Xs, w.f.ys, w.f.Zs, w.f.yypart, st);
  transpose_square(kuu_linv, p.Mp, w.R, st);
  if (p.Npad == 0) zero_slabs(p, w.f.Kfu, w.f.slab, st);
  for (auto [r0, rows] : SuperChunks{p.Npad, p.sc_rows}) {
    double* T = T_out ? T_out + (size_t)r0 * p.Mp : w.T;
    timing_begin(TIMING_ASSEMBLE, st);
    stream_assemble(p, kernel_id, w.f.Xs, w.f.ys, w.f.Zs, r0, rows, N, M, w.f.Kfu, w.f.bpart, st);
    timing_end(TIMING_ASSEMBLE, st);
    GemmDesc g;
    g.A = w.f.Kfu; g.lda = p.Mp; g.B = w.R; g.ldb = p.Mp; g.C = T; g.ldc = p.Mp;
    g.m = (int)rows; g.n = p.Mp; g.k = p.Mp; g.khi_mask = 2;
    gemm(g, st);
    launch_tpart(T, w.f.ys, r0, rows, p.Mp, w.f.bpart, st);
    timing_begin(TIMING_SYRK, st);
    launch_syrk(cx, T, p.Mp, rows / NB, split_map(p.taper, rows / NB, p.nsplit), p.ntiles, p.nsplit, r0 > 0 ? 1 : 0, w.f.slab, st);
    timing_end(TIMING_SYRK, st);
    cx.syrk_timed_rows = rows;
  }
  finish_stats(p, w.f, p.nsplit, 1, sf2, N, M, W, u, yy, kappa, st);
  return check_launch();
}


extern "C" size_t sgp_suffstats_extended_workspace_bytes(int64_t N, int M, int d) {
  if (!stream_shape_ok(N, M, d)) return 0;
  StreamPlan p = make_stream_plan(N, M, d);
  return carve_ext(nullptr, p, p.sc_rows).bytes;
}
extern "C" int sgp_suffstats_fwd_extended(const double* X, int64_t ldx, const double* y, const double* Z, int64_t ldz,
                                          const double* inv_ls, double sf2, int64_t N, int M, int d, int kernel_id,
                                          const double* kuu_linv, int level, double* W, double* u, double* yy, double* kappa,
                                          double* Kfu_out, void* ws, size_t ws_bytes, sgp_stream_t stream) {
  return sgp_suffstats_fwd_extended_ex(X, ldx, y, Z, ldz, inv_ls, sf2, N, M, d, kernel_id, kuu_linv, level, W, u, yy, kappa, Kfu_out,
                                       nullptr, ws, ws_bytes, stream);
}
extern "C" int sgp_suffstats_fwd_extended_ex(const double* X, int64_t ldx, const double* y, const double* Z, int64_t ldz,
                                             const double* inv_ls, double sf2, int64_t N, int M, int d, int kernel_id,
                                             const double* kuu_linv, int level, double* W, double* u, double* yy, double* kappa,
                                             double* Kfu_out, double* phi_diag, void* ws, size_t ws_bytes, sgp_stream_t stream) {
  return sgp_suffstats_fwd_extended_f16(X, ldx, y, Z, ldz, inv_ls, sf2, N, M, d, kernel_id, kuu_linv, level, W, u, yy, kappa, Kfu_out, nullptr,
                                        phi_diag, ws, ws_bytes, stream);
}
extern "C" int sgp_suffstats_fwd_extended_f16(const double* X, int64_t ldx, const double* y, const double* Z, int64_t ldz,
                                              const double* inv_ls, double sf2, int64_t N, int M, int d, int kernel_id,
                                              const double* kuu_linv, int level, double* W, double* u, double* yy, double* kappa,
                                              double* Kfu_out, uint16_t* Kfu_f16_out, double* phi_diag, void* ws, size_t ws_bytes,
                                              sgp_stream_t stream) {
  if ((Kfu_f16_out && !Kfu_out) || level < 1 || level > 2) return SGP_ERR_ARG;
  if (const int bad = check_stream_args({Z, inv_ls, kuu_linv, W, u, yy, kappa}, X, ldx, y, ldz, N, M, d, kernel_id, false)) return bad;
  StreamPlan p = make_stream_plan(N, M, d);
  const int64_t qrows = p.sc_rows;
  ExtWs w = carve_ext(ws, p, qrows);
  if (!ws || ws_bytes < w.bytes) return SGP_ERR_WORKSPACE;
  hipStream_t st = (hipStream_t)stream;
  stream_prologue(p, make_kern_args(inv_ls, sf2, d), X, ldx, y, Z, ldz, N, M, w.Xs, w.ys, w.Zs, w.yypart, st);
  const int ns = i8_nsplit(qrows > 0 ? qrows : 1, p.Mp);
  const size_t nslab = (size_t)ns * p.ntiles * TILE * TILE;
  if (p.Npad == 0) {
    fill_zero(w.slab, nslab, st);
    fill_zero(w.slab_lo, nslab, st);
  }
  for (auto [r0, rows] : SuperChunks{p.Npad, qrows}) {
    timing_begin(TIMING_ASSEMBLE, st);
    i8_assemble(p, kernel_id, w.Xs, w.ys, w.Zs, r0, rows, N, M, w.Q, Kfu_out ? Kfu_out + (size_t)r0 * p.Mp : nullptr, w.bpart, st,
                Kfu_f16_out ? Kfu_f16_out + (size_t)r0 * p.Mp : nullptr);
    timing_end(TIMING_ASSEMBLE, st);
    timing_begin(TIMING_SYRK, st);
    if (i8_contract(w.Q, p.Mp, rows, ns, r0 > 0 ? 1 : 0, w.slab, st, w.slab_lo, level) != SGP_OK) return SGP_ERR_LAUNCH;
    timing_end(TIMING_SYRK, st);
  }
  const int nb32 = p.Mp / 32;
  reduce_phi_dd_kernel<<<nb32 * (nb32 + 1) / 2, 256, 0, st>>>(w.slab, w.slab_lo, ns, p.ntiles, p.Mp, w.Ph, w.Pl);
  dd_launch(w.Ph, w.Pl, kuu_linv, p.Mp, w.Yh, w.Yl, 1, st, 2, 0);
  dd_launch(w.Yh, w.Yl, kuu_linv, p.Mp, w.Wh, w.Wl, 0, st, 2, 1);
  ext_w_out_kernel<<<1024, 256, 0, st>>>(w.Wh, w.Wl, M, p.Mp, sf2 * sf2, W);
  if (phi_diag) ext_phi_diag_kernel<<<(M + 255) / 256, 256, 0, st>>>(w.Ph, M, p.Mp, sf2 * sf2, phi_diag);
  fill_zero(w.bpad, p.Mp, st);
  finish_b(p, w, 1, sf2, N, M, w.bpad, yy, kappa, st);
  gemv(kuu_linv, p.Mp, p.Mp, false, w.bpad, w.upad, st);
  crop_copy(w.upad, 1, u, 1, M, 1, st);
  return check_launch();
}
```

### generalised-gaussian-processes_amd/csrc/sgp_suffstats_i8.hip

```cpp
#include <atomic>
#include "sgp_common.hpp"
#include "sgp_stream.hpp"
#include "sgp_ctx.hpp"
#include <cstdlib>
#include <type_traits>

namespace sgp {

typedef int i4v __attribute__((ext_vector_type(4)));
typedef int i16v __attribute__((ext_vector_type(16)));

constexpr int I8_NP = 7;
constexpr int I8_TR = 128, I8_TC = 64;
constexpr int I8_SCOLS = I8_TR + I8_TC;
constexpr int I8_STAGE_BYTES = 2 * I8_NP * I8_SCOLS * 16;
constexpr int I8_NSTAGE = 3;
constexpr int I8_PIECES = 2 * I8_NP * 3;
constexpr int I8_PPW = (I8_PIECES + 7) / 8;
constexpr int I8_LDS_BYTES = I8_NSTAGE * I8_STAGE_BYTES;

template <int DP, int KID, bool WK>
__global__ __launch_bounds__(256) void kfu_digits_kernel(const double* __restrict__ Xs, const double* __restrict__ ys,
                                                         const double* __restrict__ Zs, int64_t row0, int64_t N, int M, int Mp,
                                                         uint8_t* __restrict__ Q, double* __restrict__ Kfu, uint16_t* __restrict__ Kh,
                                                         double* __restrict__ bpart) {
  __shared__ double xs[ASM_ROWS][DP];
  __shared__ double ysh[ASM_ROWS];
  __shared__ double etab[EXP_TAB_N];
  const int64_t rbase = (int64_t)blockIdx.x * ASM_ROWS;
  {
    const double* src = Xs + (row0 + rbase) * DP;
    double* dst = &xs[0][0];
    for (int e = threadIdx.x; e < ASM_ROWS * DP; e += 256) dst[e] = src[e];
    ysh[threadIdx.x] = ys[row0 + rbase + threadIdx.x];
    sgp_exp_tab_load(etab);
  }
  __syncthreads();
  const int m = blockIdx.y * 256 + threadIdx.x;
  if (m >= Mp) return;
  const double zmask = m < M ? 1.0 : 0.0;
  double zr[DP];
#pragma unroll
  for (int j = 0; j < DP; ++j) zr[j] = Zs[(size_t)m * DP + j];

  constexpr unsigned long long C = 0x0080808080808080ULL;
  double bacc = 0.0;
#ifdef SGP_AB_DIGITS_NO_INTERIOR
  const bool interior = false;
#else
  const bool interior = (row0 + rbase + ASM_ROWS <= N) && ((int)(blockIdx.y * 256 + 255) < M);
#endif
  auto run = [&](auto masked_tag) {
  constexpr bool MASKED = decltype(masked_tag)::value;
  for (int g = 0; g < ASM_ROWS / 16; ++g) {
    unsigned lo[16], hi[16];
#pragma unroll
    for (int e = 0; e < 16; ++e) {
      const int i = g * 16 + e;
      const int64_t n = row0 + rbase + i;
      double r2 = 0.0;
#pragma unroll
      for (int j = 0; j < DP; ++j) {
        const double df = xs[i][j] - zr[j];
        r2 = fma(df, df, r2);
      }
      double kv = kprofile_tab<KID>(r2, etab);
      if constexpr (MASKED) kv *= (n < N ? zmask : 0.0);
      bacc = fma(kv, ysh[i], bacc);
      if constexpr (WK) {
        __builtin_nontemporal_store(kv, &Kfu[(rbase + i) * Mp + m]);
        if (Kh) {
          float kf = (float)kv;
          asm volatile("" : "+v"(kf));
          Kh[(rbase + i) * Mp + m] = __builtin_bit_cast(uint16_t, (_Float16)kf);
        }
      }
      const double th = fma(kv, 0x1p22, 0x1p52);
      const double hf = th - 0x1p52;
      const double tl = fma(-hf, 0x1p32, kv * 0x1p54) + 0x1.8p52;
      const unsigned long long tb = (unsigned long long)__double_as_longlong(tl);
      const unsigned q_hi = (unsigned)__double_as_longlong(th) - ((unsigned)(tb >> 32) & 1u);
      const unsigned long long q = ((unsigned long long)q_hi << 32) | (unsigned)tb;
      const unsigned long long qq = (q + C) ^ C;
      lo[e] = (unsigned)qq;
      hi[e] = (unsigned)(qq >> 32);
    }
    const size_t rb = (size_t)(rbase / 16 + g);
    i4v plane[8];
#pragma unroll
    for (int j = 0; j < 4; ++j) {
#pragma unroll
      for (int h = 0; h < 2; ++h) {
        const unsigned* s4 = (h ? hi : lo) + 4 * j;
        const unsigned u0 = __builtin_amdgcn_perm(s4[1], s4[0], 0x05010400u), u1 = __builtin_amdgcn_perm(s4[1], s4[0], 0x07030602u);
        const unsigned v0 = __builtin_amdgcn_perm(s4[3], s4[2], 0x05010400u), v1 = __builtin_amdgcn_perm(s4[3], s4[2], 0x07030602u);
        plane[4 * h + 0][j] = (int)__builtin_amdgcn_perm(v0, u0, 0x05040100u);
        plane[4 * h + 1][j] = (int)__builtin_amdgcn_perm(v0, u0, 0x07060302u);
        plane[4 * h + 2][j] = (int)__builtin_amdgcn_perm(v1, u1, 0x05040100u);
        if (h == 0) plane[3][j] = (int)__builtin_amdgcn_perm(v1, u1, 0x07060302u);
      }
    }
#pragma unroll
    for (int p = 0; p < I8_NP; ++p)
      __builtin_nontemporal_store(plane[p], reinterpret_cast<i4v*>(Q + ((rb * I8_NP + p) * Mp + m) * 16));
  }
  };
  if (interior) run(std::false_type{}); else run(std::true_type{});
  bpart[((row0 + rbase) / ASM_ROWS) * Mp + m] = bacc;
}

constexpr int I8_PSPLIT = 5;
#ifdef SGP_AB_I8_PAIRS34
constexpr int I8_MINSUM_DEFAULT = 5;
#else
constexpr int I8_MINSUM_DEFAULT = 6;
#endif
static_assert(2 * I8_PPW - 1 <= I8_PSPLIT * (I8_PSPLIT + 1) / 2, "every DMA piece must find its MFMA in the first half");

template <bool ACT, int I8_MINSUM, bool DD>
__device__ __forceinline__ void i8_tile_loop(uint8_t* lds, const uint8_t* __restrict__ Q, int Mp, int64_t c0, int64_t c1, int I0,
                                             int J0, int accumulate, double* __restrict__ out, size_t lo_off, int wave, int lane, int prio) {
  constexpr int I8_NG = 13 - I8_MINSUM;
  const int grp = wave >> 2, w4 = wave & 3;
  const int wi = (w4 >> 1) * 2 + grp, wj = w4 & 1;
  const int l32 = lane & 31, lh = lane >> 5;
  i16v acc[I8_NG];
#pragma unroll
  for (int g = 0; g < I8_NG; ++g)
#pragma unroll
    for (int r = 0; r < 16; ++r) acc[g][r] = 0;

  unsigned goff[I8_PPW];
  int soff[I8_PPW];
#pragma unroll
  for (int k = 0; k < I8_PPW; ++k) {
    int e = wave + 8 * k;
    if (e >= I8_PIECES) e -= I8_PIECES;
    const int rbl = e / (I8_NP * 3), rem = e % (I8_NP * 3), p = rem / 3, cg = rem % 3;
    const int col = cg < 2 ? I0 + cg * 64 : J0;
    goff[k] = (unsigned)(((rbl * I8_NP + p) * Mp + col + lane) * 16);
    soff[k] = __builtin_amdgcn_readfirstlane(((rbl * I8_NP + p) * I8_SCOLS + cg * 64) * 16);
  }
  const size_t gstride = (size_t)2 * I8_NP * Mp * 16;
  auto dma_piece = [&](const uint8_t* gbase, int sbase, int k) {
    __builtin_amdgcn_global_load_lds((const __attribute__((address_space(1))) void*)(gbase + goff[k]),
                                     (__attribute__((address_space(3))) void*)(lds + sbase + soff[k]), 16, 0, 0);
  };
  const int64_t nst = c1 - c0;
  auto wait_stage = [&](int64_t sE) {
    if (sE + 1 >= nst)
      __builtin_amdgcn_s_waitcnt(0 | (7 << 4) | (15 << 8));
    else
      __builtin_amdgcn_s_waitcnt((I8_PPW & 15) | ((I8_PPW >> 4) << 14) | (7 << 4) | (15 << 8));
  };
  auto bar = [&]() {
    __builtin_amdgcn_s_barrier();
    asm volatile("" ::: "memory");
  };
  i4v b[I8_NP], a[I8_NP];
  auto reads = [&](int64_t sidx) {
    if (ACT) {
      const uint8_t* sb = lds + (int)(sidx % I8_NSTAGE) * I8_STAGE_BYTES + lh * (I8_NP * I8_SCOLS * 16);
#pragma unroll
      for (int p = 0; p < I8_NP; ++p) {
        b[I8_NP - 1 - p] = *reinterpret_cast<const i4v*>(sb + ((I8_NP - 1 - p) * I8_SCOLS + I8_TR + wj * 32 + l32) * 16);
        a[p] = *reinterpret_cast<const i4v*>(sb + (p * I8_SCOLS + wi * 32 + l32) * 16);
      }
    }
    __builtin_amdgcn_sched_barrier(0);
  };
  auto half = [&](int p0, int p1, bool dma_on, int64_t sE) {
    if (prio) { if (dma_on) __builtin_amdgcn_s_setprio(1); else __builtin_amdgcn_s_setprio(0); }
    const bool pre = dma_on && sE + 2 < nst;
    const uint8_t* gnext = Q + (size_t)(c0 + sE + 2) * gstride;
    const int snext = (int)((sE + 2) % I8_NSTAGE) * I8_STAGE_BYTES;
    int issued = 0, kpiece = 0;
#pragma unroll
    for (int p = p0; p < p1; ++p)
#pragma unroll
      for (int r = (I8_MINSUM - p > 0 ? I8_MINSUM - p : 0); r < I8_NP; ++r) {
        if (ACT) acc[p + r - I8_MINSUM] = __builtin_amdgcn_mfma_i32_32x32x32_i8(a[p], b[r], acc[p + r - I8_MINSUM], 0, 0, 0);
        ++issued;
        if (dma_on && (issued & 1) && kpiece < I8_PPW) {
          __builtin_amdgcn_sched_barrier(0);
          if (pre) dma_piece(gnext, snext, kpiece);
          __builtin_amdgcn_sched_barrier(0);
          ++kpiece;
        }
      }
  };
  if (nst > 0) {
#pragma unroll
    for (int k = 0; k < I8_PPW; ++k) dma_piece(Q + (size_t)c0 * gstride, 0, k);
    if (nst > 1) {
#pragma unroll
      for (int k = 0; k < I8_PPW; ++k) dma_piece(Q + (size_t)(c0 + 1) * gstride, I8_STAGE_BYTES, k);
    }
    if (grp == 0) {
      for (int64_t sidx = 0; sidx < nst; ++sidx) {
        wait_stage(sidx);
        bar();
        reads(sidx);
        half(0, I8_PSPLIT, true, sidx);
        bar();
        half(I8_PSPLIT, I8_NP, false, sidx);
      }
      wait_stage(nst);
      bar();
    } else {
      wait_stage(0);
      bar();
      for (int64_t sidx = 0; sidx < nst; ++sidx) {
        bar();
        reads(sidx);
        half(0, I8_PSPLIT, true, sidx);
        __builtin_amdgcn_s_waitcnt(15 | (3 << 14) | (7 << 4) | (0 << 8));
        wait_stage(sidx + 1);
        bar();
        half(I8_PSPLIT, I8_NP, false, sidx + 1);
      }
    }
  }
  if (ACT) {
#pragma unroll
    for (int r = 0; r < 16; ++r) {
      const int row = wi * 32 + (r >> 2) * 8 + lh * 4 + (r & 3);
      double* dst = out + row * TILE + wj * 32 + l32;
      if constexpr (DD) {
#pragma clang fp contract(off)
        double hi = 0.0, lo = 0.0;
        if (accumulate) { hi = dst[0]; lo = dst[lo_off]; }
#pragma unroll
        for (int g = 0; g < I8_NG; ++g) {
          const double t = (double)acc[g][r] * __builtin_ldexp(1.0, 8 * (g + I8_MINSUM) - 108);
          const double sum = hi + t;
          const double z = sum - hi;
          lo += (hi - (sum - z)) + (t - z);
          hi = sum;
        }
        const double sum = hi + lo;
        dst[lo_off] = lo - (sum - hi);
        dst[0] = sum;
      } else {
        double v = 0.0;
#pragma unroll
        for (int g = 0; g < I8_NG; ++g) v = fma((double)acc[g][r], __builtin_ldexp(1.0, 8 * (g + I8_MINSUM) - 108), v);
        *dst = accumulate ? *dst + v : v;
      }
    }
  }
}

template <int MINSUM, bool DD>
__global__ __launch_bounds__(512, 1) void i8_syrk_tile_kernel(const uint8_t* __restrict__ Q, int Mp, int64_t nsteps, int nsplit,
                                                              int ntiles, int ntiles128, int accumulate, double* __restrict__ slab,
                                                              size_t lo_off, int prio) {
  extern __shared__ __attribute__((aligned(16))) uint8_t i8_lds[];
  const int id = blockIdx.x;
  const int xcd = id & 7, jj = id >> 3;
  const int t = jj % ntiles, split = (jj / ntiles) * 8 + xcd;
  if (split >= nsplit) return;
  int ti = (int)((sqrtf(4.0f * t + 1.0f) - 1.0f) * 0.5f);
  while ((ti + 1) * (ti + 2) <= t) ++ti;
  while (ti * (ti + 1) > t) --ti;
  const int tj = t - ti * (ti + 1);
  const int I0 = ti * I8_TR, J0 = tj * I8_TC;
  int64_t c0, c1;
  i8_split_steps(nsteps, nsplit, split, c0, c1);
  const int lane = threadIdx.x & 63;
  const int wave = __builtin_amdgcn_readfirstlane(threadIdx.x >> 6);
  double* out = slab + ((size_t)split * ntiles128 + (ti * (ti + 1) / 2 + (tj >> 1))) * (TILE * TILE) + (tj & 1) * I8_TC;
  const int grp = wave >> 2, w4 = wave & 3;
  const int wi = (w4 >> 1) * 2 + grp, wj = w4 & 1;
  if (J0 + 32 * wj <= I0 + 32 * wi + 31)
    i8_tile_loop<true, MINSUM, DD>(i8_lds, Q, Mp, c0, c1, I0, J0, accumulate, out, lo_off, wave, lane, prio);
  else
    i8_tile_loop<false, MINSUM, DD>(i8_lds, Q, Mp, c0, c1, I0, J0, accumulate, out, lo_off, wave, lane, prio);
}

template <int DP, bool WK>
static void launch_digits(int kid, dim3 grid, hipStream_t st, const double* Xs, const double* ys, const double* Zs, int64_t row0,
                          int64_t N, int M, int Mp, uint8_t* Q, double* Kfu, uint16_t* Kh, double* bpart) {
  switch (kid) {
    case SGP_KERNEL_RBF: kfu_digits_kernel<DP, SGP_KERNEL_RBF, WK><<<grid, 256, 0, st>>>(Xs, ys, Zs, row0, N, M, Mp, Q, Kfu, Kh, bpart); break;
    case SGP_KERNEL_MATERN32: kfu_digits_kernel<DP, SGP_KERNEL_MATERN32, WK><<<grid, 256, 0, st>>>(Xs, ys, Zs, row0, N, M, Mp, Q, Kfu, Kh, bpart); break;
    default: kfu_digits_kernel<DP, SGP_KERNEL_MATERN52, WK><<<grid, 256, 0, st>>>(Xs, ys, Zs, row0, N, M, Mp, Q, Kfu, Kh, bpart); break;
  }
}
template <bool WK>
static void launch_digits_dp(int DP, int kid, dim3 grid, hipStream_t st, const double* Xs, const double* ys, const double* Zs,
                             int64_t row0, int64_t N, int M, int Mp, uint8_t* Q, double* Kfu, uint16_t* Kh, double* bpart) {
  dispatch_dp(DP, [&](auto dp) { launch_digits<decltype(dp)::value, WK>(kid, grid, st, Xs, ys, Zs, row0, N, M, Mp, Q, Kfu, Kh, bpart); });
}

void i8_assemble(const StreamPlan& p, int kid, const double* Xs, const double* ys, const double* Zs, int64_t row0, int64_t rows,
                 int64_t N, int M, uint8_t* Q, double* Kfu, double* bpart, hipStream_t st, uint16_t* Kh) {
  dim3 grid((unsigned)(rows / ASM_ROWS), (p.Mp + 255) / 256);
  if (Kfu)
    launch_digits_dp<true>(p.DP, kid, grid, st, Xs, ys, Zs, row0, N, M, p.Mp, Q, Kfu, Kh, bpart);
  else
    launch_digits_dp<false>(p.DP, kid, grid, st, Xs, ys, Zs, row0, N, M, p.Mp, Q, nullptr, nullptr, bpart);
}

int i8_contract(const uint8_t* Q, int Mp, int64_t rows, int nsplit, int accumulate, double* slab, hipStream_t st, double* slab_lo, int level) {
  Ctx& cx = cur_ctx();
  static std::atomic<bool> attr_done[64];
  int dev = 0;
  if (hipGetDevice(&dev) != hipSuccess || dev < 0) return SGP_ERR_LAUNCH;
  if (dev >= 64 || !attr_done[dev].load(std::memory_order_acquire)) {
    if (hipFuncSetAttribute((const void*)i8_syrk_tile_kernel<I8_MINSUM_DEFAULT, false>, hipFuncAttributeMaxDynamicSharedMemorySize,
                            I8_LDS_BYTES) != hipSuccess ||
        hipFuncSetAttribute((const void*)i8_syrk_tile_kernel<5, true>, hipFuncAttributeMaxDynamicSharedMemorySize, I8_LDS_BYTES) !=
            hipSuccess ||
        hipFuncSetAttribute((const void*)i8_syrk_tile_kernel<4, true>, hipFuncAttributeMaxDynamicSharedMemorySize, I8_LDS_BYTES) !=
            hipSuccess)
      return SGP_ERR_LAUNCH;
    if (dev < 64) attr_done[dev].store(true, std::memory_order_release);
  }
  const int nrt = Mp / I8_TR, ntiles = nrt * (nrt + 1), ntiles128 = nrt * (nrt + 1) / 2;
  const int prio = cx.i8_prio;
  if (slab_lo && level >= 2)
    i8_syrk_tile_kernel<4, true><<<nsplit * ntiles, 512, I8_LDS_BYTES, st>>>(Q, Mp, rows / 32, nsplit, ntiles, ntiles128, accumulate, slab,
                                                                             (size_t)(slab_lo - slab), prio);
  else if (slab_lo)
    i8_syrk_tile_kernel<5, true><<<nsplit * ntiles, 512, I8_LDS_BYTES, st>>>(Q, Mp, rows / 32, nsplit, ntiles, ntiles128, accumulate, slab,
                                                                             (size_t)(slab_lo - slab), prio);
  else
    i8_syrk_tile_kernel<I8_MINSUM_DEFAULT, false><<<nsplit * ntiles, 512, I8_LDS_BYTES, st>>>(Q, Mp, rows / 32, nsplit, ntiles, ntiles128,
                                                                                               accumulate, slab, 0, prio);
  return SGP_OK;
}

}
```

### generalised-gaussian-processes_amd/engine.py

```python
from __future__ import annotations

import ctypes as C
from typing import Optional, Sequence

import numpy as np
import torch

from . import _lib
from ._lib import COMP_LEN, KERNEL_IDS, OUT_LEN

RESULT_HEAD = OUT_LEN + 4


def _kernel_id(kernel) -> int:
    if isinstance(kernel, int):
        if kernel not in KERNEL_IDS.values():
            raise ValueError("unknown kernel id %r" % (kernel,))
        return kernel
    try:
        return KERNEL_IDS[str(kernel).lower()]
    except KeyError:
        raise ValueError("unknown kernel %r (expected one of %s)" % (kernel, sorted(KERNEL_IDS))) from None


def _likelihood_id(likelihood) -> int:
    name = "bernoulli" if likelihood == "bernoulli_probit" else likelihood
    if name not in _lib.LIKELIHOOD_IDS:
        raise ValueError("unknown likelihood %r (known: %s)" % (likelihood, ", ".join(sorted(_lib.LIKELIHOOD_IDS))))
    return _lib.LIKELIHOOD_IDS[name]


class HipEngine:

    OPTIONS = {"contraction": _lib.OPT_CONTRACTION, "asm_overlap": _lib.OPT_ASM_OVERLAP, "kfu_budget_bytes": _lib.OPT_KFU_BUDGET_BYTES,
               "cond_limit": _lib.OPT_COND_LIMIT, "cu_budget": _lib.OPT_CU_BUDGET, "timing": _lib.OPT_TIMING,
               "shared_device": _lib.OPT_SHARED_DEVICE}

    def __init__(self, device: Optional[torch.device] = None, own_context: bool = False):
        self.lib = _lib.load_library()
        if not torch.cuda.is_available():
            raise _lib.SgpLibraryError("HipEngine needs a HIP device (torch.cuda.is_available() is False); "
                                       "there is no CPU implementation of the sparse-GP core")
        self.device = torch.device(device) if device is not None else torch.device("cuda", torch.cuda.current_device())
        self._ws = {}
        self._ctx = None
        if own_context:
            self._ctx = self.lib.sgp_ctx_create(self.device.index if self.device.index is not None else torch.cuda.current_device())
            if not self._ctx:
                raise _lib.SgpLibraryError("sgp_ctx_create failed")

    def __del__(self):
        ctx, self._ctx = getattr(self, "_ctx", None), None
        if ctx:
            try:
                self.lib.sgp_ctx_destroy(C.c_void_p(ctx))
            except Exception:
                pass

    class _ContextFree:

        def __init__(self, eng):
            self._eng = eng

        def __getattr__(self, name):
            eng = self._eng
            fn = getattr(eng.lib, name)
            if not eng._ctx:
                return fn
            bind = eng.lib.sgp_ctx_bind_thread

            def call(*a):
                bind(C.c_void_p(eng._ctx))
                try:
                    return fn(*a)
                finally:
                    bind(C.c_void_p(0))
            return call

    @property
    def _cf(self):
        cf = self.__dict__.get("_cf_obj")
        if cf is None:
            cf = self.__dict__["_cf_obj"] = HipEngine._ContextFree(self)
        return cf

    def _c(self):
        return C.c_void_p(self._ctx) if self._ctx else C.c_void_p(0)

    def set_option(self, name: str, value) -> float:
        prev = self.lib.sgp_ctx_get_option(self._c(), self.OPTIONS[name])
        _lib.check("sgp_ctx_set_option", self.lib.sgp_ctx_set_option(self._c(), self.OPTIONS[name], float(value)))
        return prev

    def get_option(self, name: str) -> float:
        return self.lib.sgp_ctx_get_option(self._c(), self.OPTIONS[name])

    def contraction_last(self) -> int:
        return int(self.lib.sgp_ctx_contraction_last(self._c()))

    def would_use_i8(self, N: int, M: int) -> bool:
        return bool(self.lib.sgp_ctx_contraction_would_use_i8(self._c(), int(N), int(M)))

    def _workspace(self, name: str, nbytes: int) -> torch.Tensor:
        buf = self._ws.get(name)
        if buf is None or buf.numel() < nbytes:
            buf = torch.empty(max(int(nbytes), 256), dtype=torch.uint8, device=self.device)
            self._ws[name] = buf
        return buf

    def _stream(self, stream=None):
        return C.c_void_p((stream if stream is not None else torch.cuda.current_stream(self.device)).cuda_stream)

    def _chk(self, t: torch.Tensor, name: str) -> torch.Tensor:
        if t.dtype != torch.float64 or t.device != self.device or not t.is_contiguous():
            raise ValueError("%s must be a contiguous float64 tensor on %s (got %s, %s)" % (name, self.device, t.dtype, t.device))
        return t

    @staticmethod
    def hyper_len(kernel, d: int) -> int:
        return COMP_LEN if _kernel_id(kernel) == KERNEL_IDS["composite"] else d

    def _inv_ls(self, ls: Sequence[float], d: int, kernel="rbf"):
        c = self.__dict__.get("_ils")
        if c is not None and type(ls) is list and c[1] == d and c[2] == kernel and c[0] == ls:
            return c[3]
        vals = [float(v) for v in (ls.tolist() if hasattr(ls, "tolist") else ls)]
        if _kernel_id(kernel) == KERNEL_IDS["composite"]:
            if len(vals) != COMP_LEN:
                raise ValueError("a composite kernel takes a %d-entry parameter block (got %d)" % (COMP_LEN, len(vals)))
            arr = (C.c_double * COMP_LEN)(*vals)
        else:
            if len(vals) == 1 and d > 1:
                vals = vals * d
            if len(vals) != d:
                raise ValueError("lengthscale has %d entries, expected %d" % (len(vals), d))
            arr = (C.c_double * d)(*[1.0 / v for v in vals])
        if type(ls) is list:
            self._ils = (list(ls), d, kernel, arr)
        return arr

    @staticmethod
    def _ptr(t: Optional[torch.Tensor]):
        return C.c_void_p(t.data_ptr()) if t is not None and t.numel() > 0 else C.c_void_p(0)

    def empty(self, *shape):
        return torch.empty(*shape, dtype=torch.float64, device=self.device)

    def _pass1(self, X, y, Z, kuu_linv, out, ws_name: str, ws_query, *query_args, limits: str = ""):
        N, d = X.shape
        M = Z.shape[0]
        self._chk(Z, "Z")
        if kuu_linv is not None:
            self._chk(kuu_linv, "kuu_linv")
        if N > 0:
            self._chk(X, "X"), self._chk(y, "y")
        if out is None:
            out = self.empty(M * M + M + 2)
        nbytes = ws_query(self._c(), N, M, d, *query_args)
        if nbytes == 0:
            raise ValueError("unsupported shape N=%d M=%d d=%d%s" % (N, M, d, limits))
        base = out.data_ptr()
        stats = [C.c_void_p(base + 8 * o) for o in (0, M * M, M * M + M, M * M + M + 1)]
        return N, M, d, out, self._workspace(ws_name, nbytes), stats

    def kfu_buffer(self, N: int, M: int) -> torch.Tensor:
        return self.empty(self.lib.sgp_kfu_len(N, M))

    def kfu_f16_buffer(self, N: int, M: int) -> torch.Tensor:
        return torch.empty(self.lib.sgp_kfu_len(N, M), dtype=torch.float16, device=self.device)

    def suffstats(self, X, y, Z, ls, sf2, kernel="rbf", out: Optional[torch.Tensor] = None,
                  kfu: Optional[torch.Tensor] = None, gate: Optional[torch.cuda.Event] = None) -> torch.Tensor:
        N, M, d, out, ws, stats = self._pass1(X, y, Z, None, out, "fwd_kfu" if kfu is not None else "fwd",
                                              self.lib.sgp_ctx_suffstats_workspace_bytes, 1 if kfu is not None else 0,
                                              limits=" (d <= %d, M <= %d)" % (_lib.SGP_MAX_DIM, _lib.SGP_MAX_INDUCING))
        if gate is not None:
            self.lib.sgp_ctx_set_pass1_gate(self._c(), C.c_void_p(gate.cuda_event))
        st = self.lib.sgp_ctx_suffstats_fwd(
            self._c(), self._ptr(X), d, self._ptr(y), self._ptr(Z), d, self._inv_ls(ls, d, kernel), float(sf2), N, M, d, _kernel_id(kernel),
            *stats, self._ptr(kfu), self._ptr(ws), ws.numel(), self._stream())
        _lib.check("sgp_suffstats_fwd", st)
        return out

    def suffstats_whitened(self, X, y, Z, ls, sf2, kuu_linv, kernel="rbf", out: Optional[torch.Tensor] = None) -> torch.Tensor:
        N, M, d, out, ws, stats = self._pass1(X, y, Z, kuu_linv, out, "fwd_whitened", self.lib.sgp_ctx_suffstats_whitened_workspace_bytes)
        st = self.lib.sgp_ctx_suffstats_fwd_whitened(
            self._c(), self._ptr(X), d, self._ptr(y), self._ptr(Z), d, self._inv_ls(ls, d, kernel), float(sf2), N, M, d, _kernel_id(kernel),
            self._ptr(kuu_linv), *stats, self._ptr(ws), ws.numel(), self._stream())
        _lib.check("sgp_suffstats_fwd_whitened", st)
        return out

    def suffstats_whitened_rows(self, X, y, Z, ls, sf2, kuu_linv, kernel="rbf", out: Optional[torch.Tensor] = None,
                                t_out: Optional[torch.Tensor] = None) -> torch.Tensor:
        N, M, d, out, ws, stats = self._pass1(X, y, Z, kuu_linv, out, "fwd_whitened_rows_t" if t_out is not None else "fwd_whitened_rows",
                                              self.lib.sgp_ctx_suffstats_whitened_rows_workspace_bytes, 1 if t_out is not None else 0)
        if t_out is not None:
            self._chk(t_out, "t_out")
            if t_out.numel() < self.lib.sgp_kfu_len(N, M):
                raise ValueError("t_out holds %d doubles, sgp_kfu_len(N, M) = %d" % (t_out.numel(), self.lib.sgp_kfu_len(N, M)))
        st = self.lib.sgp_ctx_suffstats_fwd_whitened_rows(
            self._c(), self._ptr(X), d, self._ptr(y), self._ptr(Z), d, self._inv_ls(ls, d, kernel), float(sf2), N, M, d, _kernel_id(kernel),
            self._ptr(kuu_linv), *stats, self._ptr(t_out), self._ptr(ws), ws.numel(), self._stream())
        _lib.check("sgp_suffstats_fwd_whitened_rows", st)
        return out

    def suffstats_extended(self, X, y, Z, ls, sf2, kuu_linv, kernel="rbf", out: Optional[torch.Tensor] = None,
                           kfu: Optional[torch.Tensor] = None, level: int = 1, phi_diag: Optional[torch.Tensor] = None,
                           kfu_f16: Optional[torch.Tensor] = None) -> torch.Tensor:
        N, M, d, out, ws, stats = self._pass1(X, y, Z, kuu_linv, out, "fwd_extended", self.lib.sgp_ctx_suffstats_extended_workspace_bytes)
        if kfu is not None:
            self._chk(kfu, "kfu")
            if kfu.numel() < self.lib.sgp_kfu_len(N, M):
                raise ValueError("kfu holds %d doubles, sgp_kfu_len(N, M) = %d" % (kfu.numel(), self.lib.sgp_kfu_len(N, M)))
        if phi_diag is not None:
            self._chk(phi_diag, "phi_diag")
            if phi_diag.numel() < M:
                raise ValueError("phi_diag holds %d doubles, M = %d" % (phi_diag.numel(), M))
        if kfu_f16 is not None:
            if kfu is None or kfu_f16.dtype != torch.float16 or not kfu_f16.is_contiguous() or kfu_f16.device != self.device \
                    or kfu_f16.numel() < self.lib.sgp_kfu_len(N, M):
                raise ValueError("kfu_f16: a contiguous float16 tensor of sgp_kfu_len(N, M) elements on this device, together with kfu")
        st = self.lib.sgp_ctx_suffstats_fwd_extended_f16(
            self._c(), self._ptr(X), d, self._ptr(y), self._ptr(Z), d, self._inv_ls(ls, d, kernel), float(sf2), N, M, d, _kernel_id(kernel),
            self._ptr(kuu_linv), int(level), *stats, self._ptr(kfu), self._ptr(kfu_f16), self._ptr(phi_diag), self._ptr(ws), ws.numel(),
            self._stream())
        _lib.check("sgp_suffstats_fwd_extended", st)
        return out

    def phibar_dd(self, Cw: torch.Tensor, kuu_linv: torch.Tensor, s2: float, want_lo: bool = False):
        M = Cw.shape[0]
        self._chk(Cw, "Cw"), self._chk(kuu_linv, "kuu_linv")
        hi = self.empty(M, M)
        lo = self.empty(M, M) if want_lo else None
        ws = self._workspace("phibar_dd", self.lib.sgp_phibar_dd_workspace_bytes(M))
        st = self.lib.sgp_phibar_dd(self._ptr(Cw), self._ptr(kuu_linv), M, float(s2), self._ptr(hi), self._ptr(lo),
                                    self._ptr(ws), ws.numel(), self._stream())
        _lib.check("sgp_phibar_dd", st)
        return hi, lo

    def bwd_lo_supported(self, N: int, M: int, d: int, kernel="rbf") -> bool:
        return kernel == "rbf" and self.lib.sgp_suffstats_bwd_lo_workspace_bytes(int(N), int(M), int(d)) > 0

    def suffstats_bwd_lo(self, X, y, Z, ls, sf2, Phibar_lo, kfu, grads: torch.Tensor, kernel="rbf", delta: Optional[torch.Tensor] = None,
                         kfu_f16: Optional[torch.Tensor] = None) -> torch.Tensor:
        N, d = X.shape
        M = Z.shape[0]
        self._chk(Phibar_lo, "Phibar_lo")
        if kfu is not None:
            self._chk(kfu, "kfu")
        elif kfu_f16 is None:
            raise ValueError("suffstats_bwd_lo needs kfu or kfu_f16")
        if kfu_f16 is not None and (kfu_f16.dtype != torch.float16 or kfu_f16.device != self.device or kfu_f16.numel() < self.lib.sgp_kfu_len(N, M)):
            raise ValueError("kfu_f16: a float16 tensor of sgp_kfu_len(N, M) elements on this device")
        nh = self.hyper_len(kernel, d)
        ws = self._workspace("bwd_lo", self.lib.sgp_suffstats_bwd_lo_workspace_bytes_ex(N, M, d, 1 if kfu_f16 is not None else 0))
        base = grads.data_ptr()
        st = self.lib.sgp_suffstats_bwd_lo_f16(self._ptr(X), d, self._ptr(y), self._ptr(Z), d, self._inv_ls(ls, d, kernel), float(sf2),
                                               self._ptr(Phibar_lo), self._ptr(kfu), self._ptr(kfu_f16), N, M, d, _kernel_id(kernel),
                                               C.c_void_p(base), C.c_void_p(base + 8 * nh), self._ptr(delta), self._ptr(ws), ws.numel(),
                                               self._stream())
# ... 696 lines not shown
```

### include/sgp.h

```cpp
#ifndef SGP_H
#define SGP_H

#include <stddef.h>
#include <stdint.h>

#ifdef __cplusplus
extern "C" {
#endif
#if defined(__GNUC__) || defined(__clang__)
#pragma GCC visibility push(default)
#endif

typedef void* sgp_stream_t;

#define SGP_ABI_VERSION 3
#define SGP_MAX_DIM 32
#define SGP_MAX_INDUCING 4096

#define SGP_INFO_TIMEOUT (-7777)

#define SGP_KERNEL_RBF 0
#define SGP_KERNEL_MATERN32 1
#define SGP_KERNEL_MATERN52 2
#define SGP_KERNEL_COMPOSITE 3
#define SGP_COMP_MAX_TERMS 4
#define SGP_COMP_MAX_FACTORS 2
#define SGP_COMP_LEN 33
#define SGP_FAC_EXPQUAD 0
#define SGP_FAC_MATERN32 1
#define SGP_FAC_MATERN52 2
#define SGP_FAC_RATQUAD 3
#define SGP_FAC_PERIODIC 4

#define SGP_OK 0
#define SGP_ERR_ARG (-1)
#define SGP_ERR_DIM (-2)
#define SGP_ERR_WORKSPACE (-3)
#define SGP_ERR_LAUNCH (-4)

#define SGP_OUT_F 0
#define SGP_OUT_LOGMARG 1
#define SGP_OUT_TRACE 2
#define SGP_OUT_LOGDETB 3
#define SGP_OUT_QUAD 4
#define SGP_OUT_TRW 5
#define SGP_OUT_S2BAR 6
#define SGP_OUT_KAPPABAR 7
#define SGP_OUT_LEN 8

int sgp_abi_version(void);

typedef struct sgp_ctx sgp_ctx;
#define SGP_OPT_CONTRACTION 0
#define SGP_OPT_ASM_OVERLAP 1
#define SGP_OPT_KFU_BUDGET_BYTES 2
#define SGP_OPT_COND_LIMIT 3
#define SGP_OPT_CU_BUDGET 4
#define SGP_OPT_TIMING 5
#define SGP_OPT_SHARED_DEVICE 6
sgp_ctx* sgp_ctx_create(int device);
void sgp_ctx_destroy(sgp_ctx* ctx);
int sgp_ctx_device(const sgp_ctx* ctx);
int sgp_ctx_set_option(sgp_ctx* ctx, int option, double value);
double sgp_ctx_get_option(const sgp_ctx* ctx, int option);
void sgp_ctx_bind_thread(sgp_ctx* ctx);
void sgp_ctx_set_pass1_gate(sgp_ctx* ctx, void* hip_event);
int sgp_ctx_contraction_last(const sgp_ctx* ctx);
int sgp_ctx_contraction_would_use_i8(const sgp_ctx* ctx, int64_t N, int M);
int sgp_ctx_timing_last_ms(sgp_ctx* ctx, int slot, float* ms);
int64_t sgp_ctx_timing_last_rows(const sgp_ctx* ctx, int slot);
size_t sgp_ctx_suffstats_workspace_bytes(const sgp_ctx* ctx, int64_t N, int M, int d, int caller_owns_kfu);
int sgp_ctx_suffstats_fwd(sgp_ctx* ctx, const double* X, int64_t ldx, const double* y, const double* Z, int64_t ldz,
                          const double* inv_ls, double sf2, int64_t N, int M, int d, int kernel_id, double* Phi, double* b,
                          double* yy, double* kappa, double* Kfu_out, void* ws, size_t ws_bytes, sgp_stream_t stream);
int sgp_ctx_suffstats_bwd(sgp_ctx* ctx, const double* X, int64_t ldx, const double* y, const double* Z, int64_t ldz,
                          const double* inv_ls, double sf2, const double* Phibar, const double* bbar, double kappabar,
                          const double* Kfu_in, int64_t N, int M, int d, int kernel_id, double* g_ls, double* g_sf2, double* g_Z,
                          void* ws, size_t ws_bytes, sgp_stream_t stream);
int sgp_ctx_kuu_factor(sgp_ctx* ctx, const double* Kuu, int M, double* Linv_out, int* info, void* ws, size_t ws_bytes,
                       sgp_stream_t stream);
int sgp_ctx_kuu_factor_ex(sgp_ctx* ctx, const double* Kuu, int M, double* Linv_out, int* info, double* trace_out, void* ws,
                          size_t ws_bytes, sgp_stream_t stream);
int sgp_ctx_bound_from_stats(sgp_ctx* ctx, const double* Kuu, const double* Phi, const double* b, const double* yy,
                             const double* kappa, double s2, int64_t N, int M, int with_adjoints, double* out, double* Phibar,
                             double* bbar, double* Kuubar, double* factors, const double* kuu_linv, int* info, void* ws,
                             size_t ws_bytes, sgp_stream_t stream);
size_t sgp_ctx_suffstats_whitened_workspace_bytes(const sgp_ctx* ctx, int64_t N, int M, int d);
int sgp_ctx_suffstats_fwd_whitened(sgp_ctx* ctx, const double* X, int64_t ldx, const double* y, const double* Z, int64_t ldz,
                                   const double* inv_ls, double sf2, int64_t N, int M, int d, int kernel_id, const double* kuu_linv,
                                   double* W, double* u, double* yy, double* kappa, void* ws, size_t ws_bytes, sgp_stream_t stream);
size_t sgp_ctx_suffstats_whitened_rows_workspace_bytes(const sgp_ctx* ctx, int64_t N, int M, int d, int caller_owns_t);
int sgp_ctx_suffstats_fwd_whitened_rows(sgp_ctx* ctx, const double* X, int64_t ldx, const double* y, const double* Z, int64_t ldz,
                                        const double* inv_ls, double sf2, int64_t N, int M, int d, int kernel_id,
                                        const double* kuu_linv, double* W, double* u, double* yy, double* kappa, double* T_out,
                                        void* ws, size_t ws_bytes, sgp_stream_t stream);
size_t sgp_ctx_suffstats_extended_workspace_bytes(const sgp_ctx* ctx, int64_t N, int M, int d);
int sgp_ctx_suffstats_fwd_extended(sgp_ctx* ctx, const double* X, int64_t ldx, const double* y, const double* Z, int64_t ldz,
                                   const double* inv_ls, double sf2, int64_t N, int M, int d, int kernel_id, const double* kuu_linv,
                                   int level, double* W, double* u, double* yy, double* kappa, double* Kfu_out, double* phi_diag,
                                   void* ws, size_t ws_bytes, sgp_stream_t stream);
size_t sgp_ctx_suffstats_bwd_factored_workspace_bytes(const sgp_ctx* ctx, int64_t N, int M, int d, int caller_owns_t);
int sgp_ctx_suffstats_bwd_factored(sgp_ctx* ctx, const double* X, int64_t ldx, const double* y, const double* Z, int64_t ldz,
                                   const double* inv_ls, double sf2, const double* kuu_linv, const double* Cw, double s2,
                                   const double* bbar, double kappabar, int64_t N, int M, int d, int kernel_id, const double* T_in,
                                   double* g_ls, double* g_sf2, double* g_Z, void* ws, size_t ws_bytes, sgp_stream_t stream);
int sgp_ctx_bound_from_whitened_stats(sgp_ctx* ctx, const double* W, const double* u, const double* yy, const double* kappa, double s2,
                                      int64_t N, int M, int with_adjoints, double* out, double* Phibar, double* bbar, double* Kuubar,
                                      double* factors, const double* kuu_linv, int* info, double* Cw, void* ws, size_t ws_bytes,
                                      sgp_stream_t stream);
int sgp_ctx_mixture_predict(sgp_ctx* ctx, const double* X, int64_t ldx, const double* y, int64_t N, const double* Xs, int64_t ldxs,
                            int64_t T, const double* Z, int64_t ldz, int S, const double* inv_ls, const double* sf2, const double* s2,
                            double jitter, int M, int d, int kernel_id, int pred_noise, double gate_jitter, double* mean, double* var,
                            double* cov, int* info, int* gate_info, void* ws, size_t ws_bytes, sgp_stream_t stream);
int sgp_ctx_mixture_predict_zs(sgp_ctx* ctx, const double* X, int64_t ldx, const double* y, int64_t N, const double* Xs,
                               int64_t ldxs, int64_t T, const double* Z, int64_t ldz, int64_t z_stride, int S, const double* inv_ls,
                               const double* sf2, const double* s2, double jitter, int M, int d, int kernel_id, int pred_noise,
                               double gate_jitter, double* mean, double* var, double* cov, int* info, int* gate_info, void* ws,
                               size_t ws_bytes, sgp_stream_t stream);

void sgp_set_cu_budget(int n);
const char* sgp_status_string(int status);

void sgp_timing_enable(int on);
int sgp_timing_last_ms(int slot, float* ms);
int64_t sgp_timing_last_rows(int slot);
void sgp_set_asm_overlap(int mode);

size_t sgp_suffstats_workspace_bytes(int64_t N, int M, int d);
size_t sgp_suffstats_workspace_bytes_ex(int64_t N, int M, int d, int caller_owns_kfu);
size_t sgp_kfu_len(int64_t N, int M);
int sgp_set_contraction(int mode);
int sgp_contraction_last(void);
void sgp_set_pass1_gate(void* hip_event);

void sgp_set_kfu_budget_bytes(size_t bytes);
int sgp_suffstats_fwd(const double* X, int64_t ldx, const double* y,
                      const double* Z, int64_t ldz, const double* inv_ls, double sf2,
                      int64_t N, int M, int d, int kernel_id,
                      double* Phi, double* b, double* yy, double* kappa, double* Kfu_out,
                      void* ws, size_t ws_bytes, sgp_stream_t stream);

size_t sgp_stats_packed_len(int M);
// ... 280 lines not shown
```

Before: 70.64.

## Run backward Kbar pass on int8 digit planes with tagged Kfu handoff

Adds an int8 split-digit path for the backward pass that contracts Phibar against Kfu. Phibar is quantised into digit planes, and Kfu is either emitted as transposed int8 planes during the forward pass (tagged in the context so the backward pass recognises it) or re-assembled per superchunk. The goal is to replace the FP64 Kbar/gradient pass with integer matrix-core tiles, and to reuse the planes stored by the forward pass. This adds workspace, extra plane-writing work in the forward pass, and reconstruction-accuracy risk, and the tagging adds pointer-identity state to the context.

```diff
diff --git a/generalised-gaussian-processes_amd/_lib.py b/generalised-gaussian-processes_amd/_lib.py
--- a/generalised-gaussian-processes_amd/_lib.py
+++ b/generalised-gaussian-processes_amd/_lib.py
@@ -14,6 +14,7 @@
 SGPMC_LIK_OUT_LEN = 3
 COMP_LEN = 33
 OPT_CONTRACTION, OPT_ASM_OVERLAP, OPT_KFU_BUDGET_BYTES, OPT_COND_LIMIT, OPT_CU_BUDGET, OPT_TIMING, OPT_SHARED_DEVICE = range(7)
+OPT_PASS2_LAST, OPT_PASS2_DUMP, OPT_KFU_PLANES = 7, 8, 9
 OUT_F, OUT_LOGMARG, OUT_TRACE, OUT_LOGDETB, OUT_QUAD, OUT_TRW, OUT_S2BAR, OUT_KAPPABAR, OUT_LEN = range(9)
 
 
diff --git a/generalised-gaussian-processes_amd/core.py b/generalised-gaussian-processes_amd/core.py
--- a/generalised-gaussian-processes_amd/core.py
+++ b/generalised-gaussian-processes_amd/core.py
@@ -396,7 +396,9 @@
                     and e.would_use_i8(int(self.X.shape[0]), M)):
                 gate = ready
         try:
-            packed = e.suffstats(self.X, self.y, Z, ls, sf2, self.kernel, kfu=kfu, **({"gate": gate} if gate is not None else {}))
+            planes = kfu is not None and hasattr(e, "pass2_last")
+            packed = e.suffstats(self.X, self.y, Z, ls, sf2, self.kernel, kfu=kfu, **({"gate": gate} if gate is not None else {}),
+                                 **({"kfu_planes": True} if planes else {}))
             self._allreduce_stats(packed, M)
         finally:
             if overlap:
diff --git a/generalised-gaussian-processes_amd/csrc/sgp_ctx.hip b/generalised-gaussian-processes_amd/csrc/sgp_ctx.hip
--- a/generalised-gaussian-processes_amd/csrc/sgp_ctx.hip
+++ b/generalised-gaussian-processes_amd/csrc/sgp_ctx.hip
@@ -16,6 +16,7 @@
   c.syrk_waves = env_int("SGP_SYRK_WAVES", 4);
   c.syrk_glds = env_int("SGP_SYRK_GLDS", 0);
   c.i8_prio = env_int("SGP_I8_PRIO", 0);
+  c.i8_pass2 = env_int("SGP_I8_PASS2", 1) != 0 ? 1 : 0;
   c.shared_device = env_int("SGP_SHARED_DEVICE", 0) != 0 ? 1 : 0;
 }
 
@@ -98,6 +99,13 @@
     case SGP_OPT_SHARED_DEVICE:
       c.shared_device = value != 0.0 ? 1 : 0;
       return SGP_OK;
+    case SGP_OPT_KFU_PLANES:
+      c.kfu_planes_next = value != 0.0 ? 1 : 0;
+      return SGP_OK;
+    case SGP_OPT_PASS2_DUMP:
+      if (!(value >= 0.0 && value < 9007199254740992.0)) return SGP_ERR_ARG;
+      c.pass2_dump = reinterpret_cast<double*>((uintptr_t)value);
+      return SGP_OK;
     default:
       return SGP_ERR_ARG;
   }
@@ -113,6 +121,9 @@
     case SGP_OPT_CU_BUDGET: return (double)c.cu_budget;
     case SGP_OPT_TIMING: return (double)c.timing;
     case SGP_OPT_SHARED_DEVICE: return (double)c.shared_device;
+    case SGP_OPT_PASS2_LAST: return (double)c.pass2_used;
+    case SGP_OPT_KFU_PLANES: return (double)c.kfu_planes_next;
+    case SGP_OPT_PASS2_DUMP: return (double)(uintptr_t)c.pass2_dump;
     default: return -1.0;
   }
 }
diff --git a/generalised-gaussian-processes_amd/csrc/sgp_ctx.hpp b/generalised-gaussian-processes_amd/csrc/sgp_ctx.hpp
--- a/generalised-gaussian-processes_amd/csrc/sgp_ctx.hpp
+++ b/generalised-gaussian-processes_amd/csrc/sgp_ctx.hpp
@@ -17,9 +17,16 @@
   int timing = 0;
   int shared_device = 0;
   int syrk_skip_upper = 1, syrk_waves = 4, syrk_glds = 0, i8_prio = 0;
+  int i8_pass2 = 1;
   int contraction_used = 0;
   hipEvent_t pass1_gate = nullptr;
+  int kfu_planes_next = 0;
   int64_t syrk_timed_rows = 0;
+  int pass2_used = 0;
+  const void* kfu_tag_ptr = nullptr;
+  int64_t kfu_tag_ld = 0;
+  int kfu_tag_mp = 0;
+  double* pass2_dump = nullptr;
   hipEvent_t ev[CTX_TIMING_SLOTS][2] = {};
   int ev_ready = 0, ev_used[CTX_TIMING_SLOTS] = {0, 0, 0};
   hipStream_t side = nullptr;
diff --git a/generalised-gaussian-processes_amd/csrc/sgp_stream.hpp b/generalised-gaussian-processes_amd/csrc/sgp_stream.hpp
--- a/generalised-gaussian-processes_amd/csrc/sgp_stream.hpp
+++ b/generalised-gaussian-processes_amd/csrc/sgp_stream.hpp
@@ -22,6 +22,7 @@
   return -1;
 }
 
+struct Ctx;
 struct StreamPlan {
   int Mp, ntr, ntiles, DP;
   int64_t Npad;
@@ -32,7 +33,43 @@
   int nmb;
   int nsplit_b;
   int taper_b[4];
-};
+  int i8b_nmt;
+  int i8b_nsplit;
+  int i8b_taper[4];
+};
+
+constexpr int I8B_TR = 128, I8B_TC = 64;
+constexpr int I8B_MAX_MP = 16384;
+constexpr int I8B_TARGET_WGS = 2048;
+static inline bool i8_kbar_shape_ok(int64_t ld, int Mp, int DP) {
+  return DP <= 8 && Mp >= 128 && Mp % 128 == 0 && Mp <= I8B_MAX_MP && (int64_t)7 * 16384 * Mp < ((int64_t)1 << 31) && ld > 0 &&
+         ld % I8B_TR == 0 && (ld + 256) * 14 * 16 < ((int64_t)1 << 32);
+}
+__host__ __device__ inline void i8_kbar_wg_map(int id, int nmt, int& mt, int& split) {
+  const int xcd = id & 7, jj = id >> 3;
+  mt = jj % nmt;
+  split = (jj / nmt) * 8 + xcd;
+}
+static inline void i8_kbar_splits(int64_t rows, int Mp, int* nmt_out, int* nsplit_out, int taper[4]) {
+  const int nmt = Mp / I8B_TC;
+  const int64_t ntn = rows / I8B_TR;
+  int64_t ns = 8 * ((I8B_TARGET_WGS + 8 * nmt - 1) / (8 * nmt));
+  if (ntn / ns < 2) {
+    const int64_t one_round = 8 * ((256 + 8 * nmt - 1) / (8 * nmt));
+    if (one_round < ns) ns = one_round;
+  }
+  int64_t lim = (ntn > 0 ? ntn : 1);
+  lim = (lim + 7) / 8 * 8;
+  if (ns > lim) ns = lim;
+  taper[0] = taper[1] = taper[2] = taper[3] = 0;
+  if (ns % 32 == 0 && ntn / ns >= 8) {
+    const int B = (int)(ns / 8);
+    taper[0] = 3 * B / 4; taper[1] = B / 4; taper[2] = B / 4; taper[3] = B / 2;
+    ns = 8 * (taper[0] + taper[1] + taper[2] + taper[3]);
+  }
+  *nmt_out = nmt;
+  *nsplit_out = (int)ns;
+}
 
 static inline int64_t bpart_rows(const StreamPlan& p) { return p.Npad / ASM_ROWS > 0 ? p.Npad / ASM_ROWS * p.asm_sub : 1; }
 
@@ -146,6 +183,7 @@
     p.taper_b[0] = 3 * B / 4; p.taper_b[1] = B / 4; p.taper_b[2] = B / 4; p.taper_b[3] = B / 2;
     p.nsplit_b = 8 * (p.taper_b[0] + p.taper_b[1] + p.taper_b[2] + p.taper_b[3]);
   }
+  i8_kbar_splits(p.sc_rows, p.Mp, &p.i8b_nmt, &p.i8b_nsplit, p.i8b_taper);
   return p;
 }
 
@@ -202,7 +240,6 @@
 void stream_assemble(const StreamPlan& p, int kid, const double* Xs, const double* ys, const double* Zs, int64_t row0,
                      int64_t rows, int64_t N, int M, double* Kfu, double* bpart, hipStream_t st);
 
-struct Ctx;
 struct FwdWs {
   double *Xs, *ys, *Zs, *Kfu, *slab, *bpart, *btmp, *yypart;
   uint8_t* Q;
@@ -254,5 +291,15 @@
                  uint16_t* Kh = nullptr );
 int i8_contract(const uint8_t* Q, int Mp, int64_t rows, int nsplit, int accumulate, double* slab, hipStream_t st, double* slab_lo = nullptr,
                 int level = 1);
-
-}
+void i8_assemble_t(const StreamPlan& p, int kid, const double* Xs, const double* Zs, int64_t row0, int64_t col0, int64_t rows, int64_t ld,
+                   int64_t N, int M, uint8_t* QT, hipStream_t st);
+void i8_phibar_digits(const double* Pb, int Mp, uint8_t* PT, double* pscale, hipStream_t st);
+int i8_kbar(const StreamPlan& p, int kid, const uint8_t* QT, int64_t ld, const uint8_t* PT, const double* pscale, const double* Xs,
+            const double* ys, const double* Zs, const double* bb, double sf2, int64_t row0, int64_t rows, int64_t N, int M, int want_gz,
+            int accumulate, double* gzpart, double* glpart, double* cdump, hipStream_t st);
+bool i8_pass2_rule(const Ctx& cx, int64_t Npad, int64_t ld, int Mp, int DP);
+void kfu_tag_set(Ctx& cx, const void* ptr, int64_t ld, int Mp);
+void kfu_tag_clear(Ctx& cx, const void* ptr);
+bool kfu_tag_is_planes(const Ctx& cx, const void* ptr, int64_t ld, int Mp);
+
+}
diff --git a/generalised-gaussian-processes_amd/csrc/sgp_suffstats_bwd.hip b/generalised-gaussian-processes_amd/csrc/sgp_suffstats_bwd.hip
--- a/generalised-gaussian-processes_amd/csrc/sgp_suffstats_bwd.hip
+++ b/generalised-gaussian-processes_amd/csrc/sgp_suffstats_bwd.hip
@@ -2,6 +2,7 @@
 #include "sgp_stream.hpp"
 #include "sgp_composite.hpp"
 #include "sgp_dense.hpp"
+#include "sgp_ctx.hpp"
 #include <cstdlib>
 
 namespace sgp {
@@ -362,6 +363,8 @@
 
 struct BwdWs {
   double *Xs, *ys, *Zs, *Pb, *bb, *gzpart, *glpart, *gacc, *bpart, *yypart, *Kfu;
+  uint8_t* PT;
+  double* pscale;
   size_t bytes;
 };
 static BwdWs carve_bwd(void* ws, const StreamPlan& p, bool need_kfu) {
@@ -372,12 +375,16 @@
   w.Zs = c.take<double>((size_t)p.Mp * p.DP);
   w.Pb = c.take<double>((size_t)p.Mp * p.Mp);
   w.bb = c.take<double>((size_t)p.Mp);
-  w.gzpart = c.take<double>((size_t)p.nsplit_b * p.Mp * p.DP);
-  w.glpart = c.take<double>((size_t)p.nsplit_b * p.nmb * (p.DP + 1));
+  const size_t ns_max = p.i8b_nsplit > p.nsplit_b ? p.i8b_nsplit : p.nsplit_b;
+  const size_t np_fp64 = (size_t)p.nsplit_b * p.nmb, np_i8 = (size_t)p.i8b_nsplit * p.i8b_nmt;
+  w.gzpart = c.take<double>(ns_max * p.Mp * p.DP);
+  w.glpart = c.take<double>((np_fp64 > np_i8 ? np_fp64 : np_i8) * (p.DP + 1));
   w.gacc = c.take<double>((size_t)p.nsplit_b * p.nmb * (2 * p.DP + 1) * 256);
   w.bpart = c.take<double>((size_t)bpart_rows(p) * p.Mp);
   w.yypart = c.take<double>(256);
   w.Kfu = need_kfu ? c.take<double>((size_t)(p.sc_rows > 0 ? p.sc_rows : 1) * p.Mp) : nullptr;
+  w.PT = c.take<uint8_t>((size_t)p.Mp * p.Mp * 7);
+  w.pscale = c.take<double>((size_t)p.Mp);
   w.bytes = c.used();
   return w;
 }
@@ -405,11 +412,11 @@
 #undef SGP_BWD_ARGS
 }
 static void finish_grads(const StreamPlan& p, const BwdWs& w, const KernArgs& ka, double kappabar, int64_t N, int M, double* g_ls,
-                         double* g_sf2, double* g_Z, hipStream_t st) {
+                         double* g_sf2, double* g_Z, hipStream_t st, int nsplit = 0, int nmb = 0) {
   const int64_t tot = (int64_t)M * ka.d;
   const int rg = (int)((tot + 255) / 256 < 1024 ? (tot + 255) / 256 : 1024);
-  bwd_reduce_kernel<<<rg < 1 ? 1 : rg, 256, 0, st>>>(w.gzpart, w.glpart, p.nsplit_b, p.nmb, p.Mp, M, p.DP, ka, kappabar * (double)N, g_ls,
-                                                    g_sf2, g_Z);
+  bwd_reduce_kernel<<<rg < 1 ? 1 : rg, 256, 0, st>>>(w.gzpart, w.glpart, nsplit ? nsplit : p.nsplit_b, nsplit ? nmb : p.nmb, p.Mp, M, p.DP, ka,
+                                                    kappabar * (double)N, g_ls, g_sf2, g_Z);
 }
 
 }
@@ -453,6 +460,31 @@
   }
 
   const int want_gz = g_Z != nullptr;
+  Ctx& cx = cur_ctx();
+  const bool planes_in = kfu_tag_is_planes(cx, Kfu_in, p.Npad, p.Mp);
+  const bool use_i8 = p.Npad > 0 && (planes_in || (!Kfu_in && i8_pass2_rule(cx, p.Npad, p.sc_rows, p.Mp, p.DP)));
+  cx.pass2_used = use_i8 ? 1 : 0;
+  if (use_i8) {
+    i8_phibar_digits(w.Pb, p.Mp, w.PT, w.pscale, st);
+    for (auto [r0, rows] : SuperChunks{p.Npad, p.sc_rows}) {
+      const uint8_t* QT = reinterpret_cast<const uint8_t*>(Kfu_in);
+      int64_t ld = p.Npad;
+      if (!Kfu_in) {
+        ld = rows;
+        timing_begin(TIMING_ASSEMBLE, st);
+        i8_assemble_t(p, kernel_id, w.Xs, w.Zs, r0, 0, rows, ld, N, M, reinterpret_cast<uint8_t*>(w.Kfu), st);
+        timing_end(TIMING_ASSEMBLE, st);
+        QT = reinterpret_cast<const uint8_t*>(w.Kfu);
+      }
+      timing_begin(TIMING_KBAR, st);
+      if (i8_kbar(p, kernel_id, QT, ld, w.PT, w.pscale, w.Xs, w.ys, w.Zs, w.bb, sf2, r0, rows, N, M, want_gz, r0 > 0 ? 1 : 0, w.gzpart,
+                  w.glpart, cx.pass2_dump, st) != SGP_OK)
+        return SGP_ERR_LAUNCH;
+      timing_end(TIMING_KBAR, st);
+    }
+    finish_grads(p, w, ka, kappabar, N, M, g_ls, g_sf2, g_Z, st, p.i8b_nsplit, p.i8b_nmt);
+    return check_launch();
+  }
   if (p.Npad == 0) launch_kbar<true>(p, kernel_id, nullptr, w, sf2, 0, 0, N, M, want_gz, 0, st);
   for (auto [r0, rows] : SuperChunks{p.Npad, p.sc_rows}) {
     const double* Kfu = Kfu_in ? Kfu_in + r0 * p.Mp : nullptr;
diff --git a/generalised-gaussian-processes_amd/csrc/sgp_suffstats_fwd.hip b/generalised-gaussian-processes_amd/csrc/sgp_suffstats_fwd.hip
--- a/generalised-gaussian-processes_amd/csrc/sgp_suffstats_fwd.hip
+++ b/generalised-gaussian-processes_amd/csrc/sgp_suffstats_fwd.hip
@@ -494,6 +494,21 @@
   return Npad > 0 && (mode == 2 || (mode == 1 && (double)Npad * Mp * Mp >= I8_MIN_WORK));
 }
 
+bool i8_pass2_rule(const Ctx& cx, int64_t Npad, int64_t ld, int Mp, int DP) {
+  return cx.i8_pass2 && i8_rule(cx.contraction, Npad, Mp) && i8_kbar_shape_ok(ld, Mp, DP);
+}
+void kfu_tag_set(Ctx& cx, const void* ptr, int64_t ld, int Mp) {
+  cx.kfu_tag_ptr = ptr;
+  cx.kfu_tag_ld = ld;
+  cx.kfu_tag_mp = Mp;
+}
+void kfu_tag_clear(Ctx& cx, const void* ptr) {
+  if (ptr && cx.kfu_tag_ptr == ptr) cx.kfu_tag_ptr = nullptr;
+}
+bool kfu_tag_is_planes(const Ctx& cx, const void* ptr, int64_t ld, int Mp) {
+  return ptr && cx.kfu_tag_ptr == ptr && cx.kfu_tag_ld == ld && cx.kfu_tag_mp == Mp;
+}
+
 constexpr int BRED_G = 64;
 FwdWs carve_fwd(void* ws, const StreamPlan& p, bool need_kfu, int64_t qrows) {
   Carver c(ws);
@@ -846,6 +861,8 @@
   Ctx& cx = cur_ctx();
   hipEvent_t gate = cx.pass1_gate;
   cx.pass1_gate = nullptr;
+  const bool planes_ok = cx.kfu_planes_next != 0;
+  cx.kfu_planes_next = 0;
   if (const int bad = check_stream_args({Z, inv_ls, Phi, b, yy, kappa}, X, ldx, y, ldz, N, M, d, kernel_id, true)) return bad;
   if (kernel_id == SGP_KERNEL_COMPOSITE) {
     CompSpec cs;
@@ -869,13 +886,18 @@
   int64_t head_chunks = 0;
   const bool use_i8 = i8_rule(cx.contraction, p.Npad, p.Mp);
   cx.contraction_used = use_i8 ? 1 : 0;
+  const bool hand_planes = planes_ok && use_i8 && Kfu_out && i8_pass2_rule(cx, p.Npad, p.Npad, p.Mp, p.DP);
+  if (hand_planes) kfu_tag_set(cx, Kfu_out, p.Npad, p.Mp);
+  else kfu_tag_clear(cx, Kfu_out);
   if (!use_i8) gate = nullptr;
   if (p.Npad > 0 && !use_i8) head_block(p, p.Npad / NB, &head_ns, &head_chunks);
   if (use_i8) {
     const int ns = i8_nsplit(qrows, p.Mp);
     for (auto [r0, rows] : SuperChunks{p.Npad, qrows}) {
       timing_begin(TIMING_ASSEMBLE, st);
-      i8_assemble(p, kernel_id, w.Xs, w.ys, w.Zs, r0, rows, N, M, w.Q, Kfu_out ? Kfu_out + (size_t)r0 * p.Mp : nullptr, w.bpart, st);
+      i8_assemble(p, kernel_id, w.Xs, w.ys, w.Zs, r0, rows, N, M, w.Q, (Kfu_out && !hand_planes) ? Kfu_out + (size_t)r0 * p.Mp : nullptr,
+                  w.bpart, st);
+      if (hand_planes) i8_assemble_t(p, kernel_id, w.Xs, w.Zs, r0, r0, rows, p.Npad, N, M, reinterpret_cast<uint8_t*>(Kfu_out), st);
       timing_end(TIMING_ASSEMBLE, st);
       if (gate && hipStreamWaitEvent(st, gate, 0) != hipSuccess) return SGP_ERR_LAUNCH;
       gate = nullptr;
@@ -937,6 +959,7 @@
   if (const int bad = check_stream_args({Z, inv_ls, kuu_linv, W, u, yy, kappa}, X, ldx, y, ldz, N, M, d, kernel_id, false)) return bad;
   StreamPlan p = make_stream_plan(N, M, d);
   if (T_out) p.sc_rows = p.Npad;
+  kfu_tag_clear(cur_ctx(), T_out);
   WhRowsWs w = carve_wh_rows(ws, p, T_out != nullptr);
   if (!ws || ws_bytes < w.bytes) return SGP_ERR_WORKSPACE;
   hipStream_t st = (hipStream_t)stream;
@@ -988,6 +1011,7 @@
                                               double* Kfu_out, uint16_t* Kfu_f16_out, double* phi_diag, void* ws, size_t ws_bytes,
                                               sgp_stream_t stream) {
   if ((Kfu_f16_out && !Kfu_out) || level < 1 || level > 2) return SGP_ERR_ARG;
+  kfu_tag_clear(cur_ctx(), Kfu_out);
   if (const int bad = check_stream_args({Z, inv_ls, kuu_linv, W, u, yy, kappa}, X, ldx, y, ldz, N, M, d, kernel_id, false)) return bad;
   StreamPlan p = make_stream_plan(N, M, d);
   const int64_t qrows = p.sc_rows;
diff --git a/generalised-gaussian-processes_amd/csrc/sgp_suffstats_i8.hip b/generalised-gaussian-processes_amd/csrc/sgp_suffstats_i8.hip
--- a/generalised-gaussian-processes_amd/csrc/sgp_suffstats_i8.hip
+++ b/generalised-gaussian-processes_amd/csrc/sgp_suffstats_i8.hip
@@ -18,6 +18,37 @@
 constexpr int I8_PIECES = 2 * I8_NP * 3;
 constexpr int I8_PPW = (I8_PIECES + 7) / 8;
 constexpr int I8_LDS_BYTES = I8_NSTAGE * I8_STAGE_BYTES;
+
+__device__ __forceinline__ void i8_store_planes(const unsigned (&lo)[16], const unsigned (&hi)[16], uint8_t* __restrict__ dst,
+                                                size_t plane_stride) {
+  i4v plane[8];
+#pragma unroll
+  for (int j = 0; j < 4; ++j) {
+#pragma unroll
+    for (int h = 0; h < 2; ++h) {
+      const unsigned* s4 = (h ? hi : lo) + 4 * j;
+      const unsigned u0 = __builtin_amdgcn_perm(s4[1], s4[0], 0x05010400u), u1 = __builtin_amdgcn_perm(s4[1], s4[0], 0x07030602u);
+      const unsigned v0 = __builtin_amdgcn_perm(s4[3], s4[2], 0x05010400u), v1 = __builtin_amdgcn_perm(s4[3], s4[2], 0x07030602u);
+      plane[4 * h + 0][j] = (int)__builtin_amdgcn_perm(v0, u0, 0x05040100u);
+      plane[4 * h + 1][j] = (int)__builtin_amdgcn_perm(v0, u0, 0x07060302u);
+      plane[4 * h + 2][j] = (int)__builtin_amdgcn_perm(v1, u1, 0x05040100u);
+      if (h == 0) plane[3][j] = (int)__builtin_amdgcn_perm(v1, u1, 0x07060302u);
+    }
+  }
+#pragma unroll
+  for (int p = 0; p < I8_NP; ++p) __builtin_nontemporal_store(plane[p], reinterpret_cast<i4v*>(dst + p * plane_stride));
+}
+
+__device__ __forceinline__ unsigned long long i8_quantise(double kv) {
+  constexpr unsigned long long C = 0x0080808080808080ULL;
+  const double th = fma(kv, 0x1p22, 0x1p52);
+  const double hf = th - 0x1p52;
+  const double tl = fma(-hf, 0x1p32, kv * 0x1p54) + 0x1.8p52;
+  const unsigned long long tb = (unsigned long long)__double_as_longlong(tl);
+  const unsigned q_hi = (unsigned)__double_as_longlong(th) - ((unsigned)(tb >> 32) & 1u);
+  const unsigned long long q = ((unsigned long long)q_hi << 32) | (unsigned)tb;
+  return (q + C) ^ C;
+}
 
 template <int DP, int KID, bool WK>
 __global__ __launch_bounds__(256) void kfu_digits_kernel(const double* __restrict__ Xs, const double* __restrict__ ys,
@@ -43,7 +74,6 @@
 #pragma unroll
   for (int j = 0; j < DP; ++j) zr[j] = Zs[(size_t)m * DP + j];
 
-  constexpr unsigned long long C = 0x0080808080808080ULL;
   double bacc = 0.0;
 #ifdef SGP_AB_DIGITS_NO_INTERIOR
   const bool interior = false;
@@ -75,38 +105,104 @@
           Kh[(rbase + i) * Mp + m] = __builtin_bit_cast(uint16_t, (_Float16)kf);
         }
       }
-      const double th = fma(kv, 0x1p22, 0x1p52);
-      const double hf = th - 0x1p52;
-      const double tl = fma(-hf, 0x1p32, kv * 0x1p54) + 0x1.8p52;
-      const unsigned long long tb = (unsigned long long)__double_as_longlong(tl);
-      const unsigned q_hi = (unsigned)__double_as_longlong(th) - ((unsigned)(tb >> 32) & 1u);
-      const unsigned long long q = ((unsigned long long)q_hi << 32) | (unsigned)tb;
-      const unsigned long long qq = (q + C) ^ C;
+      const unsigned long long qq = i8_quantise(kv);
       lo[e] = (unsigned)qq;
       hi[e] = (unsigned)(qq >> 32);
     }
     const size_t rb = (size_t)(rbase / 16 + g);
-    i4v plane[8];
-#pragma unroll
-    for (int j = 0; j < 4; ++j) {
-#pragma unroll
-      for (int h = 0; h < 2; ++h) {
-        const unsigned* s4 = (h ? hi : lo) + 4 * j;
-        const unsigned u0 = __builtin_amdgcn_perm(s4[1], s4[0], 0x05010400u), u1 = __builtin_amdgcn_perm(s4[1], s4[0], 0x07030602u);
-        const unsigned v0 = __builtin_amdgcn_perm(s4[3], s4[2], 0x05010400u), v1 = __builtin_amdgcn_perm(s4[3], s4[2], 0x07030602u);
-        plane[4 * h + 0][j] = (int)__builtin_amdgcn_perm(v0, u0, 0x05040100u);
-        plane[4 * h + 1][j] = (int)__builtin_amdgcn_perm(v0, u0, 0x07060302u);
-        plane[4 * h + 2][j] = (int)__builtin_amdgcn_perm(v1, u1, 0x05040100u);
-        if (h == 0) plane[3][j] = (int)__builtin_amdgcn_perm(v1, u1, 0x07060302u);
-      }
-    }
-#pragma unroll
-    for (int p = 0; p < I8_NP; ++p)
-      __builtin_nontemporal_store(plane[p], reinterpret_cast<i4v*>(Q + ((rb * I8_NP + p) * Mp + m) * 16));
+    i8_store_planes(lo, hi, Q + (rb * I8_NP * Mp + m) * 16, (size_t)Mp * 16);
   }
   };
   if (interior) run(std::false_type{}); else run(std::true_type{});
   bpart[((row0 + rbase) / ASM_ROWS) * Mp + m] = bacc;
+}
+
+constexpr int I8T_ZROWS = 128;
+template <int DP, int KID>
+__global__ __launch_bounds__(256) void kfut_digits_kernel(const double* __restrict__ Xs, const double* __restrict__ Zs, int64_t row0,
+                                                          int64_t col0, int64_t ld, int64_t N, int M, uint8_t* __restrict__ QT) {
+  __shared__ double zs[I8T_ZROWS][DP];
+  __shared__ double etab[EXP_TAB_N];
+  const int m0 = blockIdx.y * I8T_ZROWS;
+  {
+    const double* src = Zs + (size_t)m0 * DP;
+    double* dst = &zs[0][0];
+    for (int e = threadIdx.x; e < I8T_ZROWS * DP; e += 256) dst[e] = src[e];
+    sgp_exp_tab_load(etab);
+  }
+  __syncthreads();
+  const int64_t nl = col0 + (int64_t)blockIdx.x * 256 + threadIdx.x;
+  const int64_t n = row0 + (int64_t)blockIdx.x * 256 + threadIdx.x;
+  double xr[DP];
+#pragma unroll
+  for (int j = 0; j < DP; ++j) xr[j] = Xs[n * DP + j];
+  const bool interior = (row0 + ((int64_t)blockIdx.x + 1) * 256 <= N) && (m0 + I8T_ZROWS <= M);
+  const bool nmask = n < N;
+  auto run = [&](auto masked_tag) {
+    constexpr bool MASKED = decltype(masked_tag)::value;
+    for (int g = 0; g < I8T_ZROWS / 16; ++g) {
+      unsigned lo[16], hi[16];
+#pragma unroll
+      for (int e = 0; e < 16; ++e) {
+        const int i = g * 16 + e;
+        double r2 = 0.0;
+#pragma unroll
+        for (int j = 0; j < DP; ++j) {
+          const double df = xr[j] - zs[i][j];
+          r2 = fma(df, df, r2);
+        }
+        double kv = kprofile_tab<KID>(r2, etab);
+        if constexpr (MASKED) kv *= ((nmask && m0 + i < M) ? 1.0 : 0.0);
+        const unsigned long long qq = i8_quantise(kv);
+        lo[e] = (unsigned)qq;
+        hi[e] = (unsigned)(qq >> 32);
+      }
+      const size_t rb = (size_t)(m0 / 16 + g);
+      i8_store_planes(lo, hi, QT + (rb * I8_NP * (size_t)ld + (size_t)nl) * 16, (size_t)ld * 16);
+    }
+  };
+  if (interior) run(std::false_type{}); else run(std::true_type{});
+}
+
+__global__ __launch_bounds__(256) void pt_digits_kernel(const double* __restrict__ Pb, int Mp, uint8_t* __restrict__ PT,
+                                                        double* __restrict__ pscale) {
+  __shared__ double smax[8][32];
+  __shared__ int sbad[8][32];
+  const int c = threadIdx.x & 31, part = threadIdx.x >> 5;
+  const int m = blockIdx.x * 32 + c;
+  const int rows = Mp / 8, r0 = part * rows;
+  double mx = 0.0;
+  int bad = 0;
+  for (int r = r0; r < r0 + rows; ++r) {
+    const double a = fabs(Pb[(size_t)r * Mp + m]);
+    bad |= !(a <= 1.7976931348623157e308);
+    mx = a > mx ? a : mx;
+  }
+  smax[part][c] = mx;
+  sbad[part][c] = bad;
+  __syncthreads();
+#pragma unroll
+  for (int k = 0; k < 8; ++k) {
+    mx = k == 0 ? smax[0][c] : (smax[k][c] > mx ? smax[k][c] : mx);
+    bad = k == 0 ? sbad[0][c] : (bad | sbad[k][c]);
+  }
+  int ex = 0;
+  (void)frexp(mx, &ex);
+  if (part == 0) pscale[m] = bad ? __builtin_nan("") : ldexp(1.0, ex);
+  constexpr long long C = 0x0080808080808080LL;
+  for (int g = 0; g < rows / 16; ++g) {
+    unsigned lo[16], hi[16];
+#pragma unroll
+    for (int e = 0; e < 16; ++e) {
+      const double v = Pb[(size_t)(r0 + g * 16 + e) * Mp + m];
+      const long long q = bad ? 0 : __builtin_llrint(ldexp(v, 54 - ex));
+      const unsigned long long qq = (unsigned long long)(q + C) ^ (unsigned long long)C;
+      lo[e] = (unsigned)qq;
+      hi[e] = (unsigned)(qq >> 32) & 0x00ffffffu;
+    }
+    const size_t rb = (size_t)(r0 / 16 + g);
+    i8_store_planes(lo, hi, PT + (rb * I8_NP * (size_t)Mp + m) * 16, (size_t)Mp * 16);
+  }
 }
 
 constexpr int I8_PSPLIT = 5;
@@ -117,9 +213,10 @@
 #endif
 static_assert(2 * I8_PPW - 1 <= I8_PSPLIT * (I8_PSPLIT + 1) / 2, "every DMA piece must find its MFMA in the first half");
 
-template <bool ACT, int I8_MINSUM, bool DD>
-__device__ __forceinline__ void i8_tile_loop(uint8_t* lds, const uint8_t* __restrict__ Q, int Mp, int64_t c0, int64_t c1, int I0,
-                                             int J0, int accumulate, double* __restrict__ out, size_t lo_off, int wave, int lane, int prio) {
+template <bool ACT, int I8_MINSUM, bool TWO, class Epi>
+__device__ __forceinline__ void i8_tile_loop(uint8_t* lds, const uint8_t* __restrict__ Q, int64_t ld, const uint8_t* __restrict__ QB,
+                                             int64_t ldB, int64_t c0, int64_t c1, int64_t I0, int J0, int wave, int lane, int prio,
+                                             Epi&& epi) {
   constexpr int I8_NG = 13 - I8_MINSUM;
   const int grp = wave >> 2, w4 = wave & 3;
   const int wi = (w4 >> 1) * 2 + grp, wj = w4 & 1;
@@ -132,17 +229,25 @@
 
   unsigned goff[I8_PPW];
   int soff[I8_PPW];
+  bool fromB[I8_PPW];
 #pragma unroll
   for (int k = 0; k < I8_PPW; ++k) {
     int e = wave + 8 * k;
     if (e >= I8_PIECES) e -= I8_PIECES;
     const int rbl = e / (I8_NP * 3), rem = e % (I8_NP * 3), p = rem / 3, cg = rem % 3;
-    const int col = cg < 2 ? I0 + cg * 64 : J0;
-    goff[k] = (unsigned)(((rbl * I8_NP + p) * Mp + col + lane) * 16);
+    fromB[k] = TWO && cg == 2;
+    if constexpr (TWO)
+      goff[k] = (unsigned)(((size_t)(rbl * I8_NP + p) * (size_t)(cg < 2 ? ld : ldB) + (cg < 2 ? cg * 64 : 0) + lane) * 16);
+    else
+      goff[k] = (unsigned)(((rbl * I8_NP + p) * (int)ld + (cg < 2 ? (int)I0 + cg * 64 : J0) + lane) * 16);
     soff[k] = __builtin_amdgcn_readfirstlane(((rbl * I8_NP + p) * I8_SCOLS + cg * 64) * 16);
   }
-  const size_t gstride = (size_t)2 * I8_NP * Mp * 16;
-  auto dma_piece = [&](const uint8_t* gbase, int sbase, int k) {
+  const size_t gstride = (size_t)2 * I8_NP * ld * 16;
+  const size_t gstrideB = (size_t)2 * I8_NP * ldB * 16;
+  const uint8_t* const QA0 = TWO ? Q + (size_t)I0 * 16 : Q;
+  const uint8_t* const QB0 = TWO ? QB + (size_t)J0 * 16 : Q;
+  auto dma_piece = [&](int64_t step, int sbase, int k) {
+    const uint8_t* gbase = (TWO && fromB[k]) ? QB0 + (size_t)step * gstrideB : QA0 + (size_t)step * gstride;
     __builtin_amdgcn_global_load_lds((const __attribute__((address_space(1))) void*)(gbase + goff[k]),
                                      (__attribute__((address_space(3))) void*)(lds + sbase + soff[k]), 16, 0, 0);
   };
@@ -172,7 +277,7 @@
   auto half = [&](int p0, int p1, bool dma_on, int64_t sE) {
     if (prio) { if (dma_on) __builtin_amdgcn_s_setprio(1); else __builtin_amdgcn_s_setprio(0); }
     const bool pre = dma_on && sE + 2 < nst;
-    const uint8_t* gnext = Q + (size_t)(c0 + sE + 2) * gstride;
+    const int64_t gnext = c0 + sE + 2;
     const int snext = (int)((sE + 2) % I8_NSTAGE) * I8_STAGE_BYTES;
     int issued = 0, kpiece = 0;
 #pragma unroll
@@ -191,10 +296,10 @@
   };
   if (nst > 0) {
 #pragma unroll
-    for (int k = 0; k < I8_PPW; ++k) dma_piece(Q + (size_t)c0 * gstride, 0, k);
+    for (int k = 0; k < I8_PPW; ++k) dma_piece(c0, 0, k);
     if (nst > 1) {
 #pragma unroll
-      for (int k = 0; k < I8_PPW; ++k) dma_piece(Q + (size_t)(c0 + 1) * gstride, I8_STAGE_BYTES, k);
+      for (int k = 0; k < I8_PPW; ++k) dma_piece(c0 + 1, I8_STAGE_BYTES, k);
     }
     if (grp == 0) {
       for (int64_t sidx = 0; sidx < nst; ++sidx) {
@@ -221,7 +326,14 @@
       }
     }
   }
-  if (ACT) {
+  if (ACT) epi(acc, wi, wj, l32, lh);
+}
+
+template <int I8_MINSUM, bool DD>
+__device__ __forceinline__ void i8_fold_to_slab(const i16v (&acc)[13 - I8_MINSUM], int wi, int wj, int l32, int lh, int accumulate,
+                                                double* __restrict__ out, size_t lo_off) {
+  constexpr int I8_NG = 13 - I8_MINSUM;
+  {
 #pragma unroll
     for (int r = 0; r < 16; ++r) {
       const int row = wi * 32 + (r >> 2) * 8 + lh * 4 + (r & 3);
@@ -272,10 +384,147 @@
   double* out = slab + ((size_t)split * ntiles128 + (ti * (ti + 1) / 2 + (tj >> 1))) * (TILE * TILE) + (tj & 1) * I8_TC;
   const int grp = wave >> 2, w4 = wave & 3;
   const int wi = (w4 >> 1) * 2 + grp, wj = w4 & 1;
+  auto fold = [&](const i16v (&acc)[13 - MINSUM], int ewi, int ewj, int l32, int lh) {
+    i8_fold_to_slab<MINSUM, DD>(acc, ewi, ewj, l32, lh, accumulate, out, lo_off);
+  };
   if (J0 + 32 * wj <= I0 + 32 * wi + 31)
-    i8_tile_loop<true, MINSUM, DD>(i8_lds, Q, Mp, c0, c1, I0, J0, accumulate, out, lo_off, wave, lane, prio);
+    i8_tile_loop<true, MINSUM, false>(i8_lds, Q, Mp, Q, Mp, c0, c1, I0, J0, wave, lane, prio, fold);
   else
-    i8_tile_loop<false, MINSUM, DD>(i8_lds, Q, Mp, c0, c1, I0, J0, accumulate, out, lo_off, wave, lane, prio);
+    i8_tile_loop<false, MINSUM, false>(i8_lds, Q, Mp, Q, Mp, c0, c1, I0, J0, wave, lane, prio, fold);
+}
+
+constexpr int I8K_XS_DOUBLES = I8_TR * 8 + I8_TR;
+constexpr int I8K_LDS_BYTES = I8_LDS_BYTES + I8K_XS_DOUBLES * 8;
+
+template <int DP, int KID, bool GZ>
+__global__ __launch_bounds__(512, 1) void i8_kbar_tile_kernel(const uint8_t* __restrict__ QT, int64_t ld, const uint8_t* __restrict__ PT,
+                                                              const double* __restrict__ pscale, const double* __restrict__ Xs,
+                                                              const double* __restrict__ ys, const double* __restrict__ Zs,
+                                                              const double* __restrict__ bb, double sf2, int64_t row0, int64_t ntn,
+                                                              SplitMap tmap, int64_t N, int M, int Mp, int nmt, int accumulate,
+                                                              double* __restrict__ gzpart, double* __restrict__ glpart,
+                                                              double* __restrict__ cdump, int prio) {
+  static_assert(DP <= 8, "the x block in LDS and the register budget are sized for d <= 8");
+  extern __shared__ __attribute__((aligned(16))) uint8_t i8_lds[];
+  double* const xsh = reinterpret_cast<double*>(i8_lds + I8_LDS_BYTES);
+  int mt, split;
+  i8_kbar_wg_map((int)blockIdx.x, nmt, mt, split);
+  int64_t t0, t1;
+  split_range(tmap, split, ntn, t0, t1);
+  const int J0 = mt * I8_TC;
+  const int tid = threadIdx.x, lane = tid & 63;
+  const int wave = __builtin_amdgcn_readfirstlane(tid >> 6);
+  const int grp = wave >> 2, w4 = wave & 3;
+  const int wi = (w4 >> 1) * 2 + grp, wj = w4 & 1;
+  const int m = J0 + wj * 32 + (lane & 31);
+  double zrow[DP], gl[DP], gz[DP], gs = 0.0;
+#pragma unroll
+  for (int j = 0; j < DP; ++j) {
+    zrow[j] = Zs[(size_t)m * DP + j];
+    gl[j] = 0.0;
+    gz[j] = 0.0;
+  }
+  const double bbm = bb[m], scale = pscale[m];
+  const bool mok = m < M;
+  const int nsteps = Mp / 32;
+
+  for (int64_t t = t0; t < t1; ++t) {
+    const int64_t I0 = t * I8_TR;
+    double stage[3];
+    {
+      const double* xsrc = Xs + (row0 + I0) * DP;
+      const double* ysrc = ys + row0 + I0;
+#pragma unroll
+      for (int k = 0; k < 3; ++k) {
+        const int e = tid + 512 * k;
+        stage[k] = e < I8_TR * DP ? xsrc[e] : (e < I8_TR * DP + I8_TR ? ysrc[e - I8_TR * DP] : 0.0);
+      }
+    }
+    auto epi = [&](const i16v (&acc)[7], int ewi, int ewj, int l32, int lh) {
+#pragma unroll
+      for (int k = 0; k < 3; ++k) {
+        const int e = tid + 512 * k;
+        if (e < I8_TR * DP + I8_TR) xsh[e] = stage[k];
+      }
+      __syncthreads();
+      double* const cs = reinterpret_cast<double*>(i8_lds) + tid;
+#pragma unroll
+      for (int r = 0; r < 16; ++r) {
+        double v = 0.0;
+#pragma unroll
+        for (int g = 0; g < 7; ++g) v = fma((double)acc[g][r], __builtin_ldexp(1.0, 8 * (g + 6) - 108), v);
+        cs[r * 512] = v * scale;
+      }
+#pragma unroll 2
+      for (int r = 0; r < 16; ++r) {
+        const int row = ewi * 32 + (r >> 2) * 8 + lh * 4 + (r & 3);
+        const int64_t n = row0 + I0 + row;
+        const double C = cs[r * 512];
+        if (cdump) cdump[(size_t)(I0 + row) * Mp + m] = C;
+        const double* xq = xsh + row * DP;
+        double df[DP];
+        double r2 = 0.0;
+#pragma unroll
+        for (int j = 0; j < DP; ++j) {
+          df[j] = zrow[j] - xq[j];
+          r2 = fma(df[j], df[j], r2);
+        }
+        double kp, hp;
+        kprofile_grad<KID>(r2, kp, hp);
+        const double msk = (mok && n < N) ? 1.0 : 0.0;
+        const double kbar = (2.0 * sf2 * C + bbm * xsh[I8_TR * DP + row]) * msk;
+        gs = fma(kbar, kp, gs);
+        const double E = kbar * sf2 * hp;
+#pragma unroll
+        for (int j = 0; j < DP; ++j) {
+          const double tt = E * df[j];
+          if constexpr (GZ) gz[j] += tt;
+          gl[j] = fma(tt, df[j], gl[j]);
+        }
+      }
+      __syncthreads();
+    };
+    i8_tile_loop<true, 6, true>(i8_lds, QT, ld, PT, Mp, 0, nsteps, I0, J0, wave, lane, prio, epi);
+  }
+
+  __syncthreads();
+  double* const scratch = reinterpret_cast<double*>(i8_lds);
+  if constexpr (GZ) {
+#pragma unroll
+    for (int j = 0; j < DP; ++j) {
+      __syncthreads();
+      scratch[wave * 64 + lane] = gz[j];
+      __syncthreads();
+      if (tid < I8_TC) {
+        const int cwj = tid >> 5, c32 = tid & 31;
+        double sum = 0.0;
+#pragma unroll
+        for (int cwi = 0; cwi < 4; ++cwi) {
+          const int w = (cwi & 1) * 4 + (cwi >> 1) * 2 + cwj;
+          sum += scratch[w * 64 + c32];
+          sum += scratch[w * 64 + 32 + c32];
+        }
+        double* dst = gzpart + ((size_t)split * Mp + J0 + tid) * DP + j;
+        *dst = accumulate ? *dst + sum : sum;
+      }
+    }
+  }
+  auto block_total = [&](double v, int slot) {
+    v = wave_sum(v);
+    __syncthreads();
+    if (lane == 0) scratch[wave] = v;
+    __syncthreads();
+    if (tid == 0) {
+      double* dst = glpart + ((size_t)split * nmt + mt) * (DP + 1) + slot;
+      double tot = 0.0;
+#pragma unroll
+      for (int w = 0; w < 8; ++w) tot += scratch[w];
+      *dst = accumulate ? *dst + tot : tot;
+    }
+  };
+#pragma unroll
+  for (int j = 0; j < DP; ++j) block_total(gl[j], j);
+  block_total(gs, DP);
 }
 
 template <int DP, bool WK>
@@ -331,4 +580,63 @@
   return SGP_OK;
 }
 
-}
+void i8_assemble_t(const StreamPlan& p, int kid, const double* Xs, const double* Zs, int64_t row0, int64_t col0, int64_t rows, int64_t ld,
+                   int64_t N, int M, uint8_t* QT, hipStream_t st) {
+  const dim3 grid((unsigned)(rows / 256), p.Mp / I8T_ZROWS);
+  dispatch_dp(p.DP, [&](auto dp) {
+    constexpr int DP = decltype(dp)::value;
+    switch (kid) {
+      case SGP_KERNEL_RBF: kfut_digits_kernel<DP, SGP_KERNEL_RBF><<<grid, 256, 0, st>>>(Xs, Zs, row0, col0, ld, N, M, QT); break;
+      case SGP_KERNEL_MATERN32: kfut_digits_kernel<DP, SGP_KERNEL_MATERN32><<<grid, 256, 0, st>>>(Xs, Zs, row0, col0, ld, N, M, QT); break;
+      default: kfut_digits_kernel<DP, SGP_KERNEL_MATERN52><<<grid, 256, 0, st>>>(Xs, Zs, row0, col0, ld, N, M, QT); break;
+    }
+  });
+}
+
+void i8_phibar_digits(const double* Pb, int Mp, uint8_t* PT, double* pscale, hipStream_t st) {
+  pt_digits_kernel<<<Mp / 32, 256, 0, st>>>(Pb, Mp, PT, pscale);
+}
+
+template <int DP, int KID, bool GZ>
+static int launch_i8_kbar(int dev, int grid, hipStream_t st, const uint8_t* QT, int64_t ld, const uint8_t* PT, const double* pscale,
+                          const double* Xs, const double* ys, const double* Zs, const double* bb, double sf2, int64_t row0, int64_t ntn,
+                          const SplitMap& tmap, int64_t N, int M, int Mp, int nmt, int accumulate, double* gzpart, double* glpart,
+                          double* cdump, int prio) {
+  static std::atomic<bool> attr_done[64];
+  if (dev >= 64 || !attr_done[dev].load(std::memory_order_acquire)) {
+    if (hipFuncSetAttribute((const void*)i8_kbar_tile_kernel<DP, KID, GZ>, hipFuncAttributeMaxDynamicSharedMemorySize, I8K_LDS_BYTES) !=
+        hipSuccess)
+      return SGP_ERR_LAUNCH;
+    if (dev < 64) attr_done[dev].store(true, std::memory_order_release);
+  }
+  i8_kbar_tile_kernel<DP, KID, GZ><<<grid, 512, I8K_LDS_BYTES, st>>>(QT, ld, PT, pscale, Xs, ys, Zs, bb, sf2, row0, ntn, tmap, N, M, Mp, nmt,
+                                                                      accumulate, gzpart, glpart, cdump, prio);
+  return SGP_OK;
+}
+
+int i8_kbar(const StreamPlan& p, int kid, const uint8_t* QT, int64_t ld, const uint8_t* PT, const double* pscale, const double* Xs,
+            const double* ys, const double* Zs, const double* bb, double sf2, int64_t row0, int64_t rows, int64_t N, int M, int want_gz,
+            int accumulate, double* gzpart, double* glpart, double* cdump, hipStream_t st) {
+  if (!i8_kbar_shape_ok(ld, p.Mp, p.DP)) return SGP_ERR_ARG;
+  int dev = 0;
+  if (hipGetDevice(&dev) != hipSuccess || dev < 0) return SGP_ERR_LAUNCH;
+  const int64_t ntn = rows / I8_TR;
+  const SplitMap tmap = split_map(p.i8b_taper, ntn, p.i8b_nsplit);
+  const int grid = p.i8b_nmt * p.i8b_nsplit, prio = cur_ctx().i8_prio;
+  int rc = SGP_ERR_ARG;
+#define SGP_I8K_ARGS dev, grid, st, QT, ld, PT, pscale, Xs, ys, Zs, bb, sf2, row0, ntn, tmap, N, M, p.Mp, p.i8b_nmt, accumulate, gzpart, glpart, cdump, prio
+#define SGP_I8K_LAUNCH(KID) rc = want_gz ? launch_i8_kbar<DP, KID, true>(SGP_I8K_ARGS) : launch_i8_kbar<DP, KID, false>(SGP_I8K_ARGS)
+  dispatch_dp(p.DP <= 8 ? p.DP : 8, [&](auto dp) {
+    constexpr int DP = decltype(dp)::value <= 8 ? decltype(dp)::value : 8;
+    switch (kid) {
+      case SGP_KERNEL_RBF: SGP_I8K_LAUNCH(SGP_KERNEL_RBF); break;
+      case SGP_KERNEL_MATERN32: SGP_I8K_LAUNCH(SGP_KERNEL_MATERN32); break;
+      default: SGP_I8K_LAUNCH(SGP_KERNEL_MATERN52); break;
+    }
+  });
+#undef SGP_I8K_LAUNCH
+#undef SGP_I8K_ARGS
+  return rc;
+}
+
+}
diff --git a/generalised-gaussian-processes_amd/engine.py b/generalised-gaussian-processes_amd/engine.py
--- a/generalised-gaussian-processes_amd/engine.py
+++ b/generalised-gaussian-processes_amd/engine.py
@@ -34,7 +34,7 @@
 
     OPTIONS = {"contraction": _lib.OPT_CONTRACTION, "asm_overlap": _lib.OPT_ASM_OVERLAP, "kfu_budget_bytes": _lib.OPT_KFU_BUDGET_BYTES,
                "cond_limit": _lib.OPT_COND_LIMIT, "cu_budget": _lib.OPT_CU_BUDGET, "timing": _lib.OPT_TIMING,
-               "shared_device": _lib.OPT_SHARED_DEVICE}
+               "shared_device": _lib.OPT_SHARED_DEVICE, "pass2_dump": _lib.OPT_PASS2_DUMP}
 
     def __init__(self, device: Optional[torch.device] = None, own_context: bool = False):
         self.lib = _lib.load_library()
@@ -97,6 +97,9 @@
 
     def contraction_last(self) -> int:
         return int(self.lib.sgp_ctx_contraction_last(self._c()))
+
+    def pass2_last(self) -> int:
+        return int(self.lib.sgp_ctx_get_option(self._c(), _lib.OPT_PASS2_LAST))
 
     def would_use_i8(self, N: int, M: int) -> bool:
         return bool(self.lib.sgp_ctx_contraction_would_use_i8(self._c(), int(N), int(M)))
@@ -170,12 +173,14 @@
         return torch.empty(self.lib.sgp_kfu_len(N, M), dtype=torch.float16, device=self.device)
 
     def suffstats(self, X, y, Z, ls, sf2, kernel="rbf", out: Optional[torch.Tensor] = None,
-                  kfu: Optional[torch.Tensor] = None, gate: Optional[torch.cuda.Event] = None) -> torch.Tensor:
+                  kfu: Optional[torch.Tensor] = None, gate: Optional[torch.cuda.Event] = None, kfu_planes: bool = False) -> torch.Tensor:
         N, M, d, out, ws, stats = self._pass1(X, y, Z, None, out, "fwd_kfu" if kfu is not None else "fwd",
                                               self.lib.sgp_ctx_suffstats_workspace_bytes, 1 if kfu is not None else 0,
                                               limits=" (d <= %d, M <= %d)" % (_lib.SGP_MAX_DIM, _lib.SGP_MAX_INDUCING))
         if gate is not None:
             self.lib.sgp_ctx_set_pass1_gate(self._c(), C.c_void_p(gate.cuda_event))
+        if kfu_planes and kfu is not None:
+            self.lib.sgp_ctx_set_option(self._c(), _lib.OPT_KFU_PLANES, 1.0)
         st = self.lib.sgp_ctx_suffstats_fwd(
             self._c(), self._ptr(X), d, self._ptr(y), self._ptr(Z), d, self._inv_ls(ls, d, kernel), float(sf2), N, M, d, _kernel_id(kernel),
             *stats, self._ptr(kfu), self._ptr(ws), ws.numel(), self._stream())
diff --git a/include/sgp.h b/include/sgp.h
--- a/include/sgp.h
+++ b/include/sgp.h
@@ -58,6 +58,9 @@
 #define SGP_OPT_CU_BUDGET 4
 #define SGP_OPT_TIMING 5
 #define SGP_OPT_SHARED_DEVICE 6
+#define SGP_OPT_PASS2_LAST 7
+#define SGP_OPT_KFU_PLANES 9
+#define SGP_OPT_PASS2_DUMP 8
 sgp_ctx* sgp_ctx_create(int device);
 void sgp_ctx_destroy(sgp_ctx* ctx);
 int sgp_ctx_device(const sgp_ctx* ctx);
```

New measurement: 69.90. 1.0% lower.
